# louislung/DAE_RNN_News_Recommendation

Measured on NVIDIA H100. Metric: articles/sec, higher is better.
Workload: dtype f32

## Files before the change

### dae_rnn_news_recommendation_b200/csrc/gemm_tc.cu

```cuda
#include <cuda.h>
#include <cuda_bf16.h>
#include <type_traits>
#include "common.cuh"

namespace dae {

constexpr int BLOCK_M = 128;
constexpr int BLOCK_K = 64;
constexpr int WGMMA_K = 16;
constexpr int kThreads = 384;
constexpr int kDecodeN = 128;

__device__ __forceinline__ uint32_t smem_u32(const void* p) { return (uint32_t)__cvta_generic_to_shared(p); }

__device__ __forceinline__ void mbar_init(uint64_t* bar, uint32_t count) {
  asm volatile("mbarrier.init.shared::cta.b64 [%0], %1;" ::"r"(smem_u32(bar)), "r"(count));
}
__device__ __forceinline__ void mbar_expect_tx(uint64_t* bar, uint32_t bytes) {
  asm volatile("mbarrier.arrive.expect_tx.shared::cta.b64 _, [%0], %1;" ::"r"(smem_u32(bar)), "r"(bytes) : "memory");
}
__device__ __forceinline__ void mbar_arrive(uint64_t* bar) {
  asm volatile("mbarrier.arrive.shared::cta.b64 _, [%0];" ::"r"(smem_u32(bar)) : "memory");
}
__device__ __forceinline__ bool mbar_try_wait(uint64_t* bar, uint32_t parity) {
  uint32_t ok;
  asm volatile(
      "{\n"
      ".reg .pred p;\n"
      "mbarrier.try_wait.parity.shared::cta.b64 p, [%1], %2;\n"
      "selp.u32 %0, 1, 0, p;\n"
      "}\n"
      : "=r"(ok)
      : "r"(smem_u32(bar)), "r"(parity)
      : "memory");
  return ok != 0;
}
__device__ __forceinline__ void mbar_wait(uint64_t* bar, uint32_t parity) {
  uint32_t spins = 0;
  while (!mbar_try_wait(bar, parity)) {
    if (++spins > 4096u) {
      __nanosleep(64);
      if (spins > (1u << 26)) __trap();
    }
  }
}
__device__ __forceinline__ void fence_barrier_init() { asm volatile("fence.mbarrier_init.release.cluster;" ::: "memory"); }

__device__ __forceinline__ void tma_load_2d(const CUtensorMap* map, uint64_t* bar, void* dst, int c0, int c1) {
  asm volatile(
      "cp.async.bulk.tensor.2d.shared::cluster.global.mbarrier::complete_tx::bytes [%0], [%1, {%3, %4}], [%2];" ::"r"(smem_u32(dst)),
      "l"(map), "r"(smem_u32(bar)), "r"(c0), "r"(c1)
      : "memory");
}
__device__ __forceinline__ uint32_t cluster_ctarank() { uint32_t r; asm volatile("mov.u32 %0, %%cluster_ctarank;" : "=r"(r)); return r; }
__device__ __forceinline__ void cluster_sync_all() {
  asm volatile("barrier.cluster.arrive.release.aligned;" ::: "memory");
  asm volatile("barrier.cluster.wait.acquire.aligned;" ::: "memory");
}
__device__ __forceinline__ void tma_load_2d_mc(const CUtensorMap* map, uint64_t* bar, void* dst, int c0, int c1, uint16_t cta_mask) {
  asm volatile(
      "cp.async.bulk.tensor.2d.shared::cluster.global.mbarrier::complete_tx::bytes.multicast::cluster [%0], [%1, {%3, %4}], [%2], %5;" ::"r"(
          smem_u32(dst)),
      "l"(map), "r"(smem_u32(bar)), "r"(c0), "r"(c1), "h"(cta_mask)
      : "memory");
}
__device__ __forceinline__ void mbar_arrive_cluster(uint64_t* bar, uint32_t rank) {
  uint32_t raddr;
  asm volatile("mapa.shared::cluster.u32 %0, %1, %2;" : "=r"(raddr) : "r"(smem_u32(bar)), "r"(rank));
  asm volatile("mbarrier.arrive.release.cluster.shared::cluster.b64 _, [%0];" ::"r"(raddr) : "memory");
}
__device__ __forceinline__ void mbar_wait_cluster(uint64_t* bar, uint32_t parity) {
  uint32_t spins = 0;
  for (;;) {
    uint32_t ok;
    asm volatile(
        "{\n"
        ".reg .pred p;\n"
        "mbarrier.try_wait.parity.acquire.cluster.shared::cta.b64 p, [%1], %2;\n"
        "selp.u32 %0, 1, 0, p;\n"
        "}\n"
        : "=r"(ok)
        : "r"(smem_u32(bar)), "r"(parity)
        : "memory");
    if (ok) return;
    if (++spins > 4096u) { __nanosleep(64); if (spins > (1u << 26)) __trap(); }
  }
}

__device__ __forceinline__ void prefetch_tmap(const CUtensorMap* map) {
  asm volatile("prefetch.tensormap [%0];" ::"l"(map) : "memory");
}
__device__ __forceinline__ void named_bar_sync(int id, int threads) { asm volatile("bar.sync %0, %1;" ::"r"(id), "r"(threads) : "memory"); }

__device__ __forceinline__ void wgmma_fence() { asm volatile("wgmma.fence.sync.aligned;" ::: "memory"); }
__device__ __forceinline__ void wgmma_commit() { asm volatile("wgmma.commit_group.sync.aligned;" ::: "memory"); }
template <int N>
__device__ __forceinline__ void wgmma_wait() { asm volatile("wgmma.wait_group.sync.aligned %0;" ::"n"(N) : "memory"); }

__device__ __forceinline__ uint64_t make_desc(uint32_t saddr, uint32_t lbo_bytes, uint32_t sbo_bytes) {
  uint64_t d = 0;
  d |= (uint64_t)((saddr >> 4) & 0x3FFF);
  d |= (uint64_t)((lbo_bytes >> 4) & 0x3FFF) << 16;
  d |= (uint64_t)((sbo_bytes >> 4) & 0x3FFF) << 32;
  d |= (uint64_t)1 << 62;
  return d;
}


template <int TA, int TB>
__device__ __forceinline__ void wgmma_n128(float (&d)[64], uint64_t da, uint64_t db, uint32_t scale_d) {
  asm volatile(
      "{\n"
      ".reg .pred p;\n"
      "setp.ne.b32 p, %66, 0;\n"
      "wgmma.mma_async.sync.aligned.m64n128k16.f32.bf16.bf16 "
      "{%0, %1, %2, %3, %4, %5, %6, %7, %8, %9, %10, %11, %12, %13, %14, %15, %16, %17, %18, %19, %20, %21, %22, %23, %24, %25, %26, %27, %28, %29, %30, %31, %32, %33, %34, %35, %36, %37, %38, %39, %40, %41, %42, %43, %44, %45, %46, %47, %48, %49, %50, %51, %52, %53, %54, %55, %56, %57, %58, %59, %60, %61, %62, %63}, %64, %65, p, 1, 1, %67, %68;\n"
      "}\n"
      : "+f"(d[0]), "+f"(d[1]), "+f"(d[2]), "+f"(d[3]), "+f"(d[4]), "+f"(d[5]), "+f"(d[6]), "+f"(d[7]), "+f"(d[8]), "+f"(d[9]), "+f"(d[10]), "+f"(d[11]), "+f"(d[12]), "+f"(d[13]), "+f"(d[14]), "+f"(d[15]), "+f"(d[16]), "+f"(d[17]), "+f"(d[18]), "+f"(d[19]), "+f"(d[20]), "+f"(d[21]), "+f"(d[22]), "+f"(d[23]), "+f"(d[24]), "+f"(d[25]), "+f"(d[26]), "+f"(d[27]), "+f"(d[28]), "+f"(d[29]), "+f"(d[30]), "+f"(d[31]), "+f"(d[32]), "+f"(d[33]), "+f"(d[34]), "+f"(d[35]), "+f"(d[36]), "+f"(d[37]), "+f"(d[38]), "+f"(d[39]), "+f"(d[40]), "+f"(d[41]), "+f"(d[42]), "+f"(d[43]), "+f"(d[44]), "+f"(d[45]), "+f"(d[46]), "+f"(d[47]), "+f"(d[48]), "+f"(d[49]), "+f"(d[50]), "+f"(d[51]), "+f"(d[52]), "+f"(d[53]), "+f"(d[54]), "+f"(d[55]), "+f"(d[56]), "+f"(d[57]), "+f"(d[58]), "+f"(d[59]), "+f"(d[60]), "+f"(d[61]), "+f"(d[62]), "+f"(d[63])
      : "l"(da), "l"(db), "r"(scale_d), "n"(TA), "n"(TB));
}

template <int TA, int TB>
__device__ __forceinline__ void wgmma_n64(float (&d)[32], uint64_t da, uint64_t db, uint32_t scale_d) {
  asm volatile(
      "{\n"
      ".reg .pred p;\n"
      "setp.ne.b32 p, %34, 0;\n"
      "wgmma.mma_async.sync.aligned.m64n64k16.f32.bf16.bf16 "
      "{%0, %1, %2, %3, %4, %5, %6, %7, %8, %9, %10, %11, %12, %13, %14, %15, %16, %17, %18, %19, %20, %21, %22, %23, %24, %25, %26, %27, %28, %29, %30, %31}, %32, %33, p, 1, 1, %35, %36;\n"
      "}\n"
      : "+f"(d[0]), "+f"(d[1]), "+f"(d[2]), "+f"(d[3]), "+f"(d[4]), "+f"(d[5]), "+f"(d[6]), "+f"(d[7]), "+f"(d[8]), "+f"(d[9]), "+f"(d[10]), "+f"(d[11]), "+f"(d[12]), "+f"(d[13]), "+f"(d[14]), "+f"(d[15]), "+f"(d[16]), "+f"(d[17]), "+f"(d[18]), "+f"(d[19]), "+f"(d[20]), "+f"(d[21]), "+f"(d[22]), "+f"(d[23]), "+f"(d[24]), "+f"(d[25]), "+f"(d[26]), "+f"(d[27]), "+f"(d[28]), "+f"(d[29]), "+f"(d[30]), "+f"(d[31])
      : "l"(da), "l"(db), "r"(scale_d), "n"(TA), "n"(TB));
}

struct GemmParams {
  int M, N, K;
  int k_splits;
  int stream_k;
  int atomic;
  int a_mn, b_mn;
  int a_sym_kb;
  float alpha;
  float* C;
  int64_t ldc;
  int n_store;
  int special_col;
  float* special_out;
  const int64_t* indptr; const int32_t* indices; const float* values; const int32_t* rows;
  const float* bv; const float* weight; const double* stats;
  __nv_bfloat16* dz_hi; __nv_bfloat16* dz_lo; int64_t ld_dz;
  float* row_loss_part;
  const int32_t* tile_ptr;
};

enum { EPI_STORE = 0, EPI_DECODE = 1 };

struct Sched {
  int tiles_m, tiles, kb_total, kb_per_split, n_work, stream, w, n_cta;
  long long u, u_end;
  __device__ __forceinline__ void init(const GemmParams& p, int block_n, int pair = 0) {
    const int cta = pair ? (int)(blockIdx.x >> 1) : (int)blockIdx.x;
    n_cta = pair ? (int)(gridDim.x >> 1) : (int)gridDim.x;
    tiles_m = (p.M + BLOCK_M - 1) / BLOCK_M;
    if (pair) tiles_m = (tiles_m + 1) / 2;
    tiles = tiles_m * ((p.N + block_n - 1) / block_n);
    kb_total = (p.K + BLOCK_K - 1) / BLOCK_K;
    stream = p.stream_k;
    kb_per_split = (kb_total + p.k_splits - 1) / p.k_splits;
    n_work = tiles * p.k_splits;
    w = cta;
    const long long U = (long long)tiles * kb_total;
    u = (long long)cta * U / n_cta;
    u_end = (long long)(cta + 1) * U / n_cta;
  }
  __device__ __forceinline__ bool next(int& mb, int& nb, int& kb0, int& kb1) {
    int tile;
    if (stream) {
      if (u >= u_end) return false;
      tile = (int)(u / kb_total);
      kb0 = (int)(u - (long long)tile * kb_total);
      const long long left = u_end - u;
      kb1 = (left < (long long)(kb_total - kb0)) ? kb0 + (int)left : kb_total;
      u += kb1 - kb0;
    } else {
      if (w >= n_work) return false;
      tile = w % tiles;
      kb0 = (w / tiles) * kb_per_split;
      kb1 = min(kb_total, kb0 + kb_per_split);
      w += n_cta;
    }
    mb = tile % tiles_m;
    nb = tile / tiles_m;
    return true;
  }
};

__device__ __forceinline__ uint32_t pack_bf16(float a, float b) {
  const __nv_bfloat162 v = __floats2bfloat162_rn(a, b);
  return *reinterpret_cast<const uint32_t*>(&v);
}
__device__ __forceinline__ float f_rcp(float x) { float r; asm("rcp.approx.ftz.f32 %0, %1;" : "=f"(r) : "f"(x)); return r; }
__device__ __forceinline__ float f_lg2(float x) { float r; asm("lg2.approx.ftz.f32 %0, %1;" : "=f"(r) : "f"(x)); return r; }
__device__ __forceinline__ float f_ex2(float x) { float r; asm("ex2.approx.ftz.f32 %0, %1;" : "=f"(r) : "f"(x)); return r; }
constexpr float kLog2e = 1.4426950408889634f;

template <int ACT>
__device__ __forceinline__ float act_fast(float z) {
  if (ACT == DAE_ACT_SIGMOID) return f_rcp(1.0f + f_ex2(-kLog2e * z));
  if (ACT == DAE_ACT_TANH) return 1.0f - 2.0f * f_rcp(1.0f + f_ex2(2.0f * kLog2e * z));
  return z;
}


__device__ __forceinline__ float select16(const uint32_t (&r)[16], int j) {
  uint32_t v = r[0];
#pragma unroll
  for (int k = 1; k < 16; ++k) v = (j == k) ? r[k] : v;
  return __uint_as_float(v);
}

template <int ACT, int LOSS>
__device__ __forceinline__ void decode_chunk_generic(const uint32_t (&r)[16], const float* __restrict__ bias, float sc, bool edge,
                                                     int n_lim, int nc, uint32_t (&hpk)[8], uint32_t (&lpk)[8], float& lsum) {
#pragma unroll
  for (int j2 = 0; j2 < 8; ++j2) {
    float dzp[2];
#pragma unroll
    for (int e = 0; e < 2; ++e) {
      const int j = 2 * j2 + e;
      const float z = __uint_as_float(r[j]) + bias[j];
      const float d = act_fast<ACT>(z);
      float dz, lt;
      if (LOSS == DAE_LOSS_CE) {
        const float omd = 1.0f - d;
        const float b = omd + kEps;
        lt = -f_lg2(b);
        dz = (ACT == DAE_ACT_SIGMOID) ? ((omd != 0.0f) ? sc * d : 0.0f) : sc * act_grad_from_y<ACT>(d) * f_rcp(b);
      } else {
        lt = d * d;
        dz = 2.0f * sc * d * act_grad_from_y<ACT>(d);
      }
      if (edge) { const bool in = (nc + j < n_lim); lt = in ? lt : 0.0f; dz = in ? dz : 0.0f; }
      lsum += lt;
      dzp[e] = dz;
    }
    const uint32_t hp = pack_bf16(dzp[0], dzp[1]);
    hpk[j2] = hp;
    lpk[j2] = pack_bf16(dzp[0] - __uint_as_float(hp << 16), dzp[1] - __uint_as_float(hp & 0xffff0000u));
  }
}

__device__ __forceinline__ bool decode_chunk_sigmoid_ce(const uint32_t (&r)[16], const float* __restrict__ biasc, float sc,
                                                        uint32_t (&hpk)[8], uint32_t (&lpk)[8], float& lsum) {
  bool ok = true;
#pragma unroll
  for (int g = 0; g < 4; ++g) {
    float t[4], a[4];
#pragma unroll
    for (int j = 0; j < 4; ++j) {
      t[j] = f_ex2(fmaf(__uint_as_float(r[4 * g + j]), kLog2e, biasc[4 * g + j]));
      a[j] = 1.0f + t[j];
    }
    const float p01 = a[0] * a[1], p23 = a[2] * a[3], P = p01 * p23;
    ok = ok && (P <= 22026.0f);
    const float Rs = f_rcp(P) * sc;
    lsum += f_lg2(P);
    const float r23 = Rs * p23, r01 = Rs * p01;
    const float dz0 = t[0] * (r23 * a[1]), dz1 = t[1] * (r23 * a[0]), dz2 = t[2] * (r01 * a[3]), dz3 = t[3] * (r01 * a[2]);
    const uint32_t h0 = pack_bf16(dz0, dz1), h1 = pack_bf16(dz2, dz3);
    hpk[2 * g] = h0; hpk[2 * g + 1] = h1;
    lpk[2 * g] = pack_bf16(dz0 - __uint_as_float(h0 << 16), dz1 - __uint_as_float(h0 & 0xffff0000u));
    lpk[2 * g + 1] = pack_bf16(dz2 - __uint_as_float(h1 << 16), dz3 - __uint_as_float(h1 & 0xffff0000u));
  }
  return ok;
}

template <int BLOCK_N, int TA, int TB>
__device__ __forceinline__ void mma_kblock(float (&acc)[BLOCK_N / 2], uint32_t sa_hi, uint32_t sa_lo, uint32_t sb_hi, uint32_t sb_lo,
                                           bool first) {
  constexpr uint32_t a_lbo = TA ? 8192u : 16u, b_lbo = TB ? 8192u : 16u;
  constexpr uint32_t a_step = TA ? 2048u : 32u, b_step = TB ? 2048u : 32u;
#pragma unroll
  for (int k = 0; k < BLOCK_K / WGMMA_K; ++k) {
    const uint64_t da_hi = make_desc(sa_hi + k * a_step, a_lbo, 1024), da_lo = make_desc(sa_lo + k * a_step, a_lbo, 1024);
    const uint64_t db_hi = make_desc(sb_hi + k * b_step, b_lbo, 1024), db_lo = make_desc(sb_lo + k * b_step, b_lbo, 1024);
    const uint32_t sc = (first && k == 0) ? 0u : 1u;
    if constexpr (BLOCK_N == 128) {
      wgmma_n128<TA, TB>(acc, da_lo, db_hi, sc);
      wgmma_n128<TA, TB>(acc, da_hi, db_lo, 1u);
      wgmma_n128<TA, TB>(acc, da_hi, db_hi, 1u);
    } else {
      wgmma_n64<TA, TB>(acc, da_lo, db_hi, sc);
      wgmma_n64<TA, TB>(acc, da_hi, db_lo, 1u);
      wgmma_n64<TA, TB>(acc, da_hi, db_hi, 1u);
    }
  }
}

__device__ __forceinline__ void stage_ld16(const float* src, uint32_t (&r)[16]) {
#pragma unroll
  for (int q = 0; q < 4; ++q) {
    const float4 v = reinterpret_cast<const float4*>(src)[q];
    r[4 * q] = __float_as_uint(v.x); r[4 * q + 1] = __float_as_uint(v.y); r[4 * q + 2] = __float_as_uint(v.z); r[4 * q + 3] = __float_as_uint(v.w);
  }
}

template <int BLOCK_N, int STAGES, int EPI, int ACT, int LOSS, int PAIR, int MAJ>
__global__ void __launch_bounds__(kThreads, 1) gemm_bf16x3_kernel(const __grid_constant__ CUtensorMap tm_a_hi,
                                                                   const __grid_constant__ CUtensorMap tm_a_lo,
                                                                   const __grid_constant__ CUtensorMap tm_b_hi,
                                                                   const __grid_constant__ CUtensorMap tm_b_lo,
                                                                   const __grid_constant__ CUtensorMap tm_at_hi,
                                                                   const __grid_constant__ CUtensorMap tm_at_lo,
                                                                   const GemmParams p) {
  static_assert(!PAIR || BLOCK_N == 128, "CTA pairs split the B tile into two 64-row halves");
  constexpr int A_TILE = BLOCK_M * BLOCK_K * 2;
  constexpr int B_TILE = BLOCK_N * BLOCK_K * 2;
  constexpr int STAGE_BYTES = 2 * A_TILE + 2 * B_TILE;
  constexpr int SROW = BLOCK_N + 4;
  constexpr int kParts = 2;
  constexpr int HALF_N = BLOCK_N / kParts;
  constexpr bool kFast = (EPI == EPI_DECODE) && (ACT == DAE_ACT_SIGMOID) && (LOSS == DAE_LOSS_CE);
  extern __shared__ __align__(1024) uint8_t smem_raw[];
  uint8_t* smem = reinterpret_cast<uint8_t*>((reinterpret_cast<uintptr_t>(smem_raw) + 1023) & ~(uintptr_t)1023);
  float* stg = reinterpret_cast<float*>(smem + STAGES * STAGE_BYTES);
  __shared__ __align__(8) uint64_t full_bar[STAGES], empty_bar[STAGES];
  __shared__ float s_bias[EPI == EPI_DECODE ? 2 : 1][EPI == EPI_DECODE ? BLOCK_N : 1];
  __shared__ float s_biasc[kFast ? 2 : 1][kFast ? BLOCK_N : 1];
  __shared__ __align__(16) uint8_t s_stage[EPI == EPI_DECODE ? 8 : 1][2][32][48];

  const int warp = threadIdx.x >> 5, lane = threadIdx.x & 31;
  Sched sched;
  sched.init(p, BLOCK_N, PAIR);
  const uint32_t crank = PAIR ? cluster_ctarank() : 0u;

  if (warp == 0 && lane == 0) {
    prefetch_tmap(&tm_a_hi); prefetch_tmap(&tm_a_lo); prefetch_tmap(&tm_b_hi); prefetch_tmap(&tm_b_lo);
    if (p.a_sym_kb > 0) { prefetch_tmap(&tm_at_hi); prefetch_tmap(&tm_at_lo); }
  }
  if (warp == 1 && lane == 0) {
    for (int s = 0; s < STAGES; ++s) { mbar_init(&full_bar[s], 1); mbar_init(&empty_bar[s], PAIR ? 16 : 8); }
    fence_barrier_init();
  }
  if (PAIR) cluster_sync_all(); else __syncthreads();

  if (warp == 0) {
    if (lane == 0) {
      int stage = 0; uint32_t phase = 0;
      int mb, nb, kb0, kb1;
      while (sched.next(mb, nb, kb0, kb1)) {
        for (int kb = kb0; kb < kb1; ++kb) {
          if (PAIR) mbar_wait_cluster(&empty_bar[stage], phase ^ 1); else mbar_wait(&empty_bar[stage], phase ^ 1);
          uint8_t* sa_hi = smem + stage * STAGE_BYTES;
          uint8_t* sa_lo = sa_hi + A_TILE;
          uint8_t* sb_hi = sa_lo + A_TILE;
          uint8_t* sb_lo = sb_hi + B_TILE;
          const int mt = PAIR ? mb * 2 + (int)crank : mb;
          mbar_expect_tx(&full_bar[stage], STAGE_BYTES);
          if (p.a_sym_kb > 0 && kb >= p.a_sym_kb) {
#pragma unroll
            for (int j = 0; j < BLOCK_M / 64; ++j) {
              tma_load_2d(&tm_at_hi, &full_bar[stage], sa_hi + j * 8192, mt * BLOCK_M + j * 64, (kb - p.a_sym_kb) * BLOCK_K);
              tma_load_2d(&tm_at_lo, &full_bar[stage], sa_lo + j * 8192, mt * BLOCK_M + j * 64, (kb - p.a_sym_kb) * BLOCK_K);
            }
          } else if (!p.a_mn) {
            tma_load_2d(&tm_a_hi, &full_bar[stage], sa_hi, kb * BLOCK_K, mt * BLOCK_M);
            tma_load_2d(&tm_a_lo, &full_bar[stage], sa_lo, kb * BLOCK_K, mt * BLOCK_M);
          } else {
#pragma unroll
            for (int j = 0; j < BLOCK_M / 64; ++j) {
              tma_load_2d(&tm_a_hi, &full_bar[stage], sa_hi + j * 8192, mt * BLOCK_M + j * 64, kb * BLOCK_K);
              tma_load_2d(&tm_a_lo, &full_bar[stage], sa_lo + j * 8192, mt * BLOCK_M + j * 64, kb * BLOCK_K);
            }
          }
          const int kbb = (p.a_sym_kb > 0 && kb >= p.a_sym_kb) ? kb - p.a_sym_kb : kb;
          if (PAIR) {
            const int off = (int)crank * 8192, n_half = nb * BLOCK_N + (int)crank * 64;
            if (!p.b_mn) {
              tma_load_2d_mc(&tm_b_hi, &full_bar[stage], sb_hi + off, kbb * BLOCK_K, n_half, 0x3);
              tma_load_2d_mc(&tm_b_lo, &full_bar[stage], sb_lo + off, kbb * BLOCK_K, n_half, 0x3);
            } else {
              tma_load_2d_mc(&tm_b_hi, &full_bar[stage], sb_hi + off, n_half, kbb * BLOCK_K, 0x3);
              tma_load_2d_mc(&tm_b_lo, &full_bar[stage], sb_lo + off, n_half, kbb * BLOCK_K, 0x3);
            }
          } else if (!p.b_mn) {
            tma_load_2d(&tm_b_hi, &full_bar[stage], sb_hi, kbb * BLOCK_K, nb * BLOCK_N);
            tma_load_2d(&tm_b_lo, &full_bar[stage], sb_lo, kbb * BLOCK_K, nb * BLOCK_N);
          } else {
#pragma unroll
            for (int j = 0; j < BLOCK_N / 64; ++j) {
              tma_load_2d(&tm_b_hi, &full_bar[stage], sb_hi + j * 8192, nb * BLOCK_N + j * 64, kbb * BLOCK_K);
              tma_load_2d(&tm_b_lo, &full_bar[stage], sb_lo + j * 8192, nb * BLOCK_N + j * 64, kbb * BLOCK_K);
            }
          }
          if (++stage == STAGES) { stage = 0; phase ^= 1; }
        }
      }
    }
  } else if (warp >= 4) {
    const int wg = (warp >> 2) - 1;
    const int wi = warp & 3;
    const int quarter = wg * 2 + (wi & 1);
    const int half = wi >> 1;
    const int row_in_tile = quarter * 32 + lane;
    const int tiles_n = (p.N + BLOCK_N - 1) / BLOCK_N;
    float acc[BLOCK_N / 2];
#pragma unroll
    for (int i = 0; i < BLOCK_N / 2; ++i) acc[i] = 0.0f;
    int stage = 0; uint32_t phase = 0;
    auto release = [&](int s) {
      __syncwarp();
      if (lane == 0) { mbar_arrive(&empty_bar[s]); if (PAIR) mbar_arrive_cluster(&empty_bar[s], crank ^ 1u); }
    };
    int mb, nb, kb0, kb1;
    while (sched.next(mb, nb, kb0, kb1)) {
      if (PAIR) mb = mb * 2 + (int)crank;
      int prev = -1;
      auto run_k = [&](auto ta, auto tb, int kb_begin, int kb_end) {
        for (int kb = kb_begin; kb < kb_end; ++kb) {
          mbar_wait(&full_bar[stage], phase);
          const uint32_t sa_hi = smem_u32(smem + stage * STAGE_BYTES) + wg * 8192;
          const uint32_t sa_lo = sa_hi + A_TILE;
          const uint32_t sb_hi = smem_u32(smem + stage * STAGE_BYTES) + 2 * A_TILE, sb_lo = sb_hi + B_TILE;
          wgmma_fence();
          mma_kblock<BLOCK_N, decltype(ta)::value, decltype(tb)::value>(acc, sa_hi, sa_lo, sb_hi, sb_lo, kb == kb0);
          wgmma_commit();
          wgmma_wait<1>();
          if (prev >= 0) release(prev);
          prev = stage;
          if (++stage == STAGES) { stage = 0; phase ^= 1; }
        }
      };
      using K0 = std::integral_constant<int, 0>;
      using K1 = std::integral_constant<int, 1>;
      if (MAJ & 4) {
        run_k(K0{}, K1{}, kb0, min(kb1, p.a_sym_kb));
        run_k(K1{}, K1{}, max(kb0, p.a_sym_kb), kb1);
      } else {
        run_k(std::integral_constant<int, MAJ & 1>{}, std::integral_constant<int, (MAJ >> 1) & 1>{}, kb0, kb1);
      }
      wgmma_wait<0>();
      if (prev >= 0) release(prev);

      named_bar_sync(1 + wg, 128);
      {
        const int r0 = wg * 64 + wi * 16 + (lane >> 2), c0 = 2 * (lane & 3);
#pragma unroll
        for (int j = 0; j < BLOCK_N / 8; ++j) {
          *reinterpret_cast<float2*>(&stg[r0 * SROW + 8 * j + c0]) = make_float2(acc[4 * j], acc[4 * j + 1]);
          *reinterpret_cast<float2*>(&stg[(r0 + 8) * SROW + 8 * j + c0]) = make_float2(acc[4 * j + 2], acc[4 * j + 3]);
        }
      }
      if (EPI == EPI_DECODE) {
        for (int j = threadIdx.x - 128 * (wg + 1); j < BLOCK_N; j += 128) {
          const float b = (nb * BLOCK_N + j < p.N) ? p.bv[nb * BLOCK_N + j] : 0.0f;
          s_bias[wg][j] = b;
          if (kFast) s_biasc[wg][j] = b * kLog2e;
        }
      }
      named_bar_sync(1 + wg, 128);
      const float* srow = stg + row_in_tile * SROW + half * HALF_N;
      const int m = mb * BLOCK_M + row_in_tile;
      const int n0 = nb * BLOCK_N + half * HALF_N;

      if (EPI == EPI_STORE) {
        const float* tr = stg + (quarter * 32) * SROW + half * HALF_N;
        const int m_base = mb * BLOCK_M + quarter * 32;
        const bool vec_ok = ((p.ldc & 3) == 0) && ((reinterpret_cast<uintptr_t>(p.C) & 15) == 0);
#pragma unroll 1
        for (int c = 0; c < HALF_N / 16; ++c) {
          const int nc = n0 + c * 16;
          const bool interior = vec_ok && (m_base + 32 <= p.M) && (nc + 16 <= p.n_store) && (p.special_col < nc || p.special_col >= nc + 16);
          if (interior) {
            const int rsub = lane >> 2, c4 = (lane & 3) * 4;
            float* dst = p.C + (int64_t)(m_base + rsub) * p.ldc + nc + c4;
            const int64_t step = 8 * p.ldc;
#pragma unroll
            for (int i = 0; i < 4; ++i) {
              float4 v = *reinterpret_cast<const float4*>(&tr[(rsub + 8 * i) * SROW + c * 16 + c4]);
              v.x *= p.alpha; v.y *= p.alpha; v.z *= p.alpha; v.w *= p.alpha;
              if (p.atomic) atomicAdd(reinterpret_cast<float4*>(dst), v); else *reinterpret_cast<float4*>(dst) = v;
              dst += step;
            }
          } else {
            const int rsub = lane >> 4, csub = lane & 15;
            const int n = nc + csub;
            for (int i = 0; i < 16; ++i) {
              const int rr = 2 * i + rsub;
              const int mm = m_base + rr;
              const float v = p.alpha * tr[rr * SROW + c * 16 + csub];
              if (mm < p.M) {
                if (n == p.special_col) {
                  if (p.atomic) atomicAdd(p.special_out + mm, v); else p.special_out[mm] = v;
                } else if (n < p.n_store) {
                  float* dst = p.C + (int64_t)mm * p.ldc + n;
                  if (p.atomic) atomicAdd(dst, v); else *dst = v;
                }
              }
            }
          }
        }
      } else {
        int64_t pc = 0, pe = 0;
        int c0 = 0x7fffffff, c1 = 0x7fffffff, c2 = 0x7fffffff;
        float v0 = 0.0f, v1 = 0.0f, v2 = 0.0f;
        float sc = 0.0f;
        if (m < p.M) {
          const int64_t row = p.rows ? (int64_t)p.rows[m] : (int64_t)m;
          const int64_t rbeg = p.indptr[row];
          const int32_t* tp = p.tile_ptr + (int64_t)m * (kParts * tiles_n + 1) + nb * kParts + half;
          pc = rbeg + tp[0]; pe = rbeg + tp[1];
          if (pc < pe) { c0 = p.indices[pc]; v0 = p.values[pc]; }
          if (pc + 1 < pe) { c1 = p.indices[pc + 1]; v1 = p.values[pc + 1]; }
          if (pc + 2 < pe) { c2 = p.indices[pc + 2]; v2 = p.values[pc + 2]; }
          sc = (p.weight ? p.weight[m] : 1.0f) / ((float)p.stats[DAE_STAT_SUM_W] + kEps);
        }
        const float inv_sc = (sc != 0.0f) ? 1.0f / sc : 0.0f;
        const bool edge = (n0 + HALF_N > p.N);
        float lsum = 0.0f;
        const int ew = warp - 4;
        uint8_t* stg_hi = reinterpret_cast<uint8_t*>(&s_stage[ew][0][0][0]);
        uint8_t* stg_lo = reinterpret_cast<uint8_t*>(&s_stage[ew][1][0][0]);
        const int rsub = lane >> 1, csub = lane & 1;
        const int m_base = mb * BLOCK_M + quarter * 32;
        const int n_lim = edge ? p.N : 0x7fffffff;
#pragma unroll 1
        for (int c = 0; c < HALF_N / 16; ++c) {
          uint32_t r[16];
          stage_ld16(srow + c * 16, r);
          const int nc = n0 + c * 16;
          if (m < p.M) {
            const float* bias = &s_bias[wg][half * HALF_N + c * 16];
            uint32_t hpk[8], lpk[8];
            bool fast_ok = false;
            if (kFast && !edge) {
              const float l0 = lsum;
              fast_ok = decode_chunk_sigmoid_ce(r, &s_biasc[wg][half * HALF_N + c * 16], sc, hpk, lpk, lsum);
              if (!fast_ok) { lsum = l0; decode_chunk_generic<ACT, LOSS>(r, bias, sc, edge, n_lim, nc, hpk, lpk, lsum); }
            } else {
              decode_chunk_generic<ACT, LOSS>(r, bias, sc, edge, n_lim, nc, hpk, lpk, lsum);
            }
            uint4* sh = reinterpret_cast<uint4*>(stg_hi + lane * 48);
            uint4* sl = reinterpret_cast<uint4*>(stg_lo + lane * 48);
            sh[0] = make_uint4(hpk[0], hpk[1], hpk[2], hpk[3]); sh[1] = make_uint4(hpk[4], hpk[5], hpk[6], hpk[7]);
            sl[0] = make_uint4(lpk[0], lpk[1], lpk[2], lpk[3]); sl[1] = make_uint4(lpk[4], lpk[5], lpk[6], lpk[7]);
            while (c0 < nc + 16) {
              const float x = v0;
              const int j = c0 - nc;
              __nv_bfloat16* ph = reinterpret_cast<__nv_bfloat16*>(stg_hi + lane * 48) + j;
              __nv_bfloat16* pl = reinterpret_cast<__nv_bfloat16*>(stg_lo + lane * 48) + j;
              float d;
              if (kFast && fast_ok && sc != 0.0f) d = (__bfloat162float(*ph) + __bfloat162float(*pl)) * inv_sc;
              else d = act_fast<ACT>(select16(r, j) + bias[j]);
              const float gp = act_grad_from_y<ACT>(d);
              float dz;
              if (LOSS == DAE_LOSS_CE) {
                const float a = d + kEps, b = (1.0f - d) + kEps;
                const float la = f_lg2(a), lb = f_lg2(b);
                lsum += lb - (x * la + (1.0f - x) * lb);
                dz = sc * gp * ((1.0f - x) * f_rcp(b) - x * f_rcp(a));
              } else {
                const float e2 = x - d;
                lsum += e2 * e2 - d * d;
                dz = -2.0f * sc * e2 * gp;
              }
              const __nv_bfloat16 hb = __float2bfloat16_rn(dz);
              *ph = hb;
              *pl = __float2bfloat16_rn(dz - __bfloat162float(hb));
              ++pc;
              c0 = c1; v0 = v1; c1 = c2; v1 = v2;
              c2 = 0x7fffffff;
              if (pc + 2 < pe) { c2 = p.indices[pc + 2]; v2 = p.values[pc + 2]; }
            }
          }
          __syncwarp();
          if (nc < p.ld_dz) {
#pragma unroll
            for (int i = 0; i < 2; ++i) {
              const int rr = rsub + 16 * i;
              if (m_base + rr < p.M) {
                const int64_t off = (int64_t)(m_base + rr) * p.ld_dz + nc + csub * 8;
                *reinterpret_cast<uint4*>(p.dz_hi + off) = *reinterpret_cast<const uint4*>(stg_hi + rr * 48 + csub * 16);
                *reinterpret_cast<uint4*>(p.dz_lo + off) = *reinterpret_cast<const uint4*>(stg_lo + rr * 48 + csub * 16);
              }
            }
          }
          __syncwarp();
        }
        if (m < p.M) atomicAdd(p.row_loss_part + m, (LOSS == DAE_LOSS_CE) ? lsum * 0.6931471805599453f : lsum);
      }
    }
  }

  if (PAIR) cluster_sync_all();
}

__global__ void decode_tile_ptr_kernel(const int64_t* __restrict__ indptr, const int32_t* __restrict__ indices,
                                       const int32_t* __restrict__ rows, int M, int n_half_tiles, int half_n,
                                       int32_t* __restrict__ tile_ptr) {
  const int t = blockIdx.x * blockDim.x + threadIdx.x;
  const int m = blockIdx.y;
  if (t > n_half_tiles || m >= M) return;
  const int64_t row = rows ? (int64_t)rows[m] : (int64_t)m;
  const int64_t b = indptr[row], e = indptr[row + 1];
  const int target = t * half_n;
  int64_t lo = b, hi = e;
  while (lo < hi) { const int64_t mid = (lo + hi) >> 1; if (indices[mid] < target) lo = mid + 1; else hi = mid; }
  tile_ptr[(int64_t)m * (n_half_tiles + 1) + t] = (int32_t)(lo - b);
}

__global__ void split_bf16_kernel(const float* __restrict__ src, int rows, int cols, int64_t ld_src, __nv_bfloat16* __restrict__ hi,
                                  __nv_bfloat16* __restrict__ lo, int64_t ld_dst, int ones_col, float scale) {
  const int64_t total = (int64_t)rows * ld_dst;
  for (int64_t i = (int64_t)blockIdx.x * blockDim.x + threadIdx.x; i < total; i += (int64_t)gridDim.x * blockDim.x) {
    const int64_t r = i / ld_dst;
    const int c = (int)(i - r * ld_dst);
    float v = (c < cols) ? src[r * ld_src + c] * scale : 0.0f;
    if (c == ones_col) v = 1.0f;
    const __nv_bfloat16 h = __float2bfloat16_rn(v);
    hi[i] = h;
    lo[i] = __float2bfloat16_rn(v - __bfloat162float(h));
  }
}

__global__ void sym_split_kernel(const float* __restrict__ G, int B, int64_t ldg, float alpha, __nv_bfloat16* __restrict__ hi,
                                 __nv_bfloat16* __restrict__ lo, int64_t ld) {
  __shared__ float t[32][33];
  const int bx = blockIdx.x * 32, by = blockIdx.y * 32;
  const int tx = threadIdx.x, ty = threadIdx.y;
  for (int j = ty; j < 32; j += 8) {
    const int r = bx + j, c = by + tx;
    t[j][tx] = (r < B && c < B) ? G[(int64_t)r * ldg + c] : 0.0f;
  }
  __syncthreads();
  for (int j = ty; j < 32; j += 8) {
    const int r = by + j, c = bx + tx;
    if (r < B && c < ld) {
      float v = 0.0f;
      if (c < B) v = alpha * (G[(int64_t)r * ldg + c] + t[tx][j]);
      const __nv_bfloat16 h = __float2bfloat16_rn(v);
      hi[(int64_t)r * ld + c] = h;
      lo[(int64_t)r * ld + c] = __float2bfloat16_rn(v - __bfloat162float(h));
    }
  }
}

typedef CUresult (*PFN_encodeTiled)(CUtensorMap*, CUtensorMapDataType, cuuint32_t, void*, const cuuint64_t*, const cuuint64_t*,
                                    const cuuint32_t*, const cuuint32_t*, CUtensorMapInterleave, CUtensorMapSwizzle,
                                    CUtensorMapL2promotion, CUtensorMapFloatOOBfill);

static PFN_encodeTiled get_encode() {
  static PFN_encodeTiled fn = nullptr;
  if (!fn) {
    void* sym = nullptr;
    cudaDriverEntryPointQueryResult q;
    if (cudaGetDriverEntryPoint("cuTensorMapEncodeTiled", &sym, cudaEnableDefault, &q) == cudaSuccess && q == cudaDriverEntryPointSuccess)
      fn = reinterpret_cast<PFN_encodeTiled>(sym);
  }
  return fn;
}

static int make_map(CUtensorMap* m, const void* base, uint64_t inner, uint64_t outer, uint64_t ld, uint32_t box_outer) {
  PFN_encodeTiled enc = get_encode();
  if (!enc) { set_error("cuTensorMapEncodeTiled entry point not found"); return DAE_ERR_CUDA; }
  cuuint64_t dims[2] = {inner, outer};
  cuuint64_t strides[1] = {ld * 2};
  cuuint32_t box[2] = {64, box_outer};
  cuuint32_t estr[2] = {1, 1};
  CUresult r = enc(m, CU_TENSOR_MAP_DATA_TYPE_BFLOAT16, 2, const_cast<void*>(base), dims, strides, box, estr,
                   CU_TENSOR_MAP_INTERLEAVE_NONE, CU_TENSOR_MAP_SWIZZLE_128B, CU_TENSOR_MAP_L2_PROMOTION_L2_256B,
                   CU_TENSOR_MAP_FLOAT_OOB_FILL_NONE);
  if (r != CUDA_SUCCESS) { set_error("cuTensorMapEncodeTiled failed (%d): inner=%llu outer=%llu ld=%llu", (int)r,
                                     (unsigned long long)inner, (unsigned long long)outer, (unsigned long long)ld); return DAE_ERR_CUDA; }
  return DAE_OK;
}

struct Operand { const void* hi; const void* lo; int64_t ld; int mn_major; };

template <typename Kern>
static int ensure_smem_attr(Kern kern, int smem, bool (&done)[64]) {
  int dev = 0;
  DAE_CUDA(cudaGetDevice(&dev));
  if (dev < 0 || dev >= 64 || !done[dev]) {
    DAE_CUDA(cudaFuncSetAttribute(kern, cudaFuncAttributeMaxDynamicSharedMemorySize, smem));
    if (dev >= 0 && dev < 64) done[dev] = true;
  }
  return DAE_OK;
}


static int g_pair_mode = -1;
static int g_lean = 0;

template <int BLOCK_N, int STAGES, int EPI, int ACT, int LOSS, int PAIR, int MAJ>
static int launch_gemm_maj(const Operand& A, const Operand& B, GemmParams p, cudaStream_t st) {
  CUtensorMap ta_hi, ta_lo, tb_hi, tb_lo;
  int rc;
  constexpr int B_ROWS = PAIR ? BLOCK_N / 2 : BLOCK_N;
  if (!A.mn_major) {
    const uint64_t a_cols = p.a_sym_kb > 0 ? (uint64_t)p.M : (uint64_t)p.K;
    if ((rc = make_map(&ta_hi, A.hi, a_cols, p.M, A.ld, BLOCK_M))) return rc;
    if ((rc = make_map(&ta_lo, A.lo, a_cols, p.M, A.ld, BLOCK_M))) return rc;
  } else {
    if ((rc = make_map(&ta_hi, A.hi, p.M, p.K, A.ld, 64))) return rc;
    if ((rc = make_map(&ta_lo, A.lo, p.M, p.K, A.ld, 64))) return rc;
  }
  if (!B.mn_major) {
    if ((rc = make_map(&tb_hi, B.hi, p.K, p.N, B.ld, B_ROWS))) return rc;
    if ((rc = make_map(&tb_lo, B.lo, p.K, p.N, B.ld, B_ROWS))) return rc;
  } else {
    const uint64_t b_rows = p.a_sym_kb > 0 ? (uint64_t)p.M : (uint64_t)p.K;
    if ((rc = make_map(&tb_hi, B.hi, p.N, b_rows, B.ld, 64))) return rc;
    if ((rc = make_map(&tb_lo, B.lo, p.N, b_rows, B.ld, 64))) return rc;
  }
  p.a_mn = A.mn_major; p.b_mn = B.mn_major;
  CUtensorMap tat_hi = ta_hi, tat_lo = ta_lo;
  if (p.a_sym_kb > 0) {
    if (PAIR || A.mn_major) { set_error("dae_gemm_sym_bf16x3: unsupported configuration"); return DAE_ERR_UNSUPPORTED; }
    if ((rc = make_map(&tat_hi, A.hi, p.M, p.M, A.ld, 64))) return rc;
    if ((rc = make_map(&tat_lo, A.lo, p.M, p.M, A.ld, 64))) return rc;
  }
  constexpr int smem = STAGES * (2 * BLOCK_M * BLOCK_K * 2 + 2 * BLOCK_N * BLOCK_K * 2) + BLOCK_M * (BLOCK_N + 4) * 4 + 1024;
  int tiles_m = (p.M + BLOCK_M - 1) / BLOCK_M;
  if (PAIR) tiles_m = (tiles_m + 1) / 2;
  const int tiles_n = (p.N + BLOCK_N - 1) / BLOCK_N;
  const int kblocks = (p.K + BLOCK_K - 1) / BLOCK_K;
  auto kern = gemm_bf16x3_kernel<BLOCK_N, STAGES, EPI, ACT, LOSS, PAIR, MAJ>;
  static bool attr_done[64] = {false};
  if ((rc = ensure_smem_attr(kern, smem, attr_done))) return rc;
  const int slots = PAIR ? sm_count() / 2 : sm_count();
  int n;
  if (p.stream_k) {
    const long long units = (long long)tiles_m * tiles_n * kblocks;
    long long g = units / 6;
    if (g < 1) g = 1;
    n = (int)(g < slots ? g : slots);
  } else {
    const int items = tiles_m * tiles_n * p.k_splits;
    n = items < slots ? items : slots;
  }
  if (!PAIR) {
    kern<<<n, kThreads, smem, st>>>(ta_hi, ta_lo, tb_hi, tb_lo, tat_hi, tat_lo, p);
  } else {
    cudaLaunchConfig_t cfg{};
    cfg.gridDim = dim3(2 * n); cfg.blockDim = dim3(kThreads); cfg.dynamicSmemBytes = smem; cfg.stream = st;
    cudaLaunchAttribute at[1];
    at[0].id = cudaLaunchAttributeClusterDimension;
    at[0].val.clusterDim.x = 2; at[0].val.clusterDim.y = 1; at[0].val.clusterDim.z = 1;
    cfg.attrs = at; cfg.numAttrs = 1;
    DAE_CUDA(cudaLaunchKernelEx(&cfg, kern, ta_hi, ta_lo, tb_hi, tb_lo, tat_hi, tat_lo, p));
  }
  return DAE_OK;
}

template <int BLOCK_N, int STAGES, int EPI, int ACT, int LOSS, int PAIR>
static int launch_gemm(const Operand& A, const Operand& B, GemmParams p, cudaStream_t st) {
  if (EPI == EPI_DECODE || (!A.mn_major && !B.mn_major)) return launch_gemm_maj<BLOCK_N, STAGES, EPI, ACT, LOSS, PAIR, 0>(A, B, p, st);
  if constexpr (EPI == EPI_STORE) {
    if (A.mn_major && !B.mn_major) return launch_gemm_maj<BLOCK_N, STAGES, EPI, ACT, LOSS, PAIR, 1>(A, B, p, st);
    if (!A.mn_major) return launch_gemm_maj<BLOCK_N, STAGES, EPI, ACT, LOSS, PAIR, 2>(A, B, p, st);
    return launch_gemm_maj<BLOCK_N, STAGES, EPI, ACT, LOSS, PAIR, 3>(A, B, p, st);
  }
  return DAE_ERR_UNSUPPORTED;
}

static bool use_pair() { return g_pair_mode == 1 && !g_lean; }

}

using namespace dae;

extern "C" int dae_split_bf16(const float* src, int32_t rows, int32_t cols, int64_t ld_src, void* hi, void* lo, int64_t ld_dst,
                              int32_t ones_col, float scale, void* stream) {
  DAE_REQUIRE(src && hi && lo && rows > 0 && cols > 0 && ld_src >= cols && ld_dst >= cols, "dae_split_bf16: bad arguments");
  const int64_t total = (int64_t)rows * ld_dst;
  const int cap = sm_count() * 16;
  const int blocks = (int)((total + 255) / 256 < cap ? (total + 255) / 256 : cap);
  split_bf16_kernel<<<blocks, 256, 0, (cudaStream_t)stream>>>(src, rows, cols, ld_src, (__nv_bfloat16*)hi, (__nv_bfloat16*)lo, ld_dst,
                                                              ones_col, scale);
  DAE_CHECK_LAUNCH("dae_split_bf16");
  return DAE_OK;
}

extern "C" int dae_sym_split_bf16(const float* G, int32_t B, int64_t ldg, float alpha, void* hi, void* lo, int64_t ld, void* stream) {
  DAE_REQUIRE(G && hi && lo && B > 0 && ldg >= B && ld >= B, "dae_sym_split_bf16: bad arguments");
  dim3 grid((unsigned)((ld + 31) / 32), (B + 31) / 32), block(32, 8);
  sym_split_kernel<<<grid, block, 0, (cudaStream_t)stream>>>(G, B, ldg, alpha, (__nv_bfloat16*)hi, (__nv_bfloat16*)lo, ld);
  DAE_CHECK_LAUNCH("dae_sym_split_bf16");
  return DAE_OK;
}

extern "C" int dae_gemm_config(int32_t pair_mode, int32_t lean) {
  dae::g_pair_mode = pair_mode < 0 ? -1 : (pair_mode ? 1 : 0);
  dae::g_lean = lean ? 1 : 0;
  return DAE_OK;
}

extern "C" int dae_gemm_bf16x3(int32_t M, int32_t N, int32_t K, float alpha, const void* a_hi, const void* a_lo, int64_t lda,
                               int32_t a_mn_major, const void* b_hi, const void* b_lo, int64_t ldb, int32_t b_mn_major, float* C,
                               int64_t ldc, int32_t n_store, int32_t special_col, float* special_out, int32_t k_splits,
                               int32_t accumulate, void* stream) {
  DAE_REQUIRE(a_hi && a_lo && b_hi && b_lo && C && M > 0 && N > 0 && K > 0, "dae_gemm_bf16x3: bad arguments");
  DAE_REQUIRE(lda % 8 == 0 && ldb % 8 == 0, "dae_gemm_bf16x3: operand leading dimensions must be multiples of 8 (TMA 16-byte strides)");
  DAE_REQUIRE(((uintptr_t)a_hi | (uintptr_t)a_lo | (uintptr_t)b_hi | (uintptr_t)b_lo) % 16 == 0, "dae_gemm_bf16x3: operands must be 16-byte aligned");
  cudaStream_t st = (cudaStream_t)stream;
  if (n_store <= 0 || n_store > N) n_store = N;
  const int kblocks = (K + BLOCK_K - 1) / BLOCK_K;
  const int tm = (M + 127) / 128, tn128 = (N + 127) / 128, tn64 = (N + 63) / 64;
  const int sms = sm_count();
  int stream_k = 0;
  if (k_splits < 0) {
    const int t = tm * tn128;
    stream_k = (t % sms == 0) ? 0 : 1;
    k_splits = 1;
  }
  if (k_splits < 1) k_splits = 1;
  if (k_splits > kblocks) k_splits = kblocks;
  {
    const int per = (kblocks + k_splits - 1) / k_splits;
    k_splits = (kblocks + per - 1) / per;
  }
  const bool partial = (k_splits > 1) || stream_k;
  if (partial && !accumulate) {
    DAE_CUDA(cudaMemset2DAsync(C, ldc * sizeof(float), 0, (size_t)n_store * sizeof(float), M, st));
    if (special_col >= 0 && special_out) DAE_CUDA(cudaMemsetAsync(special_out, 0, sizeof(float) * M, st));
  }
  GemmParams p{};
  p.M = M; p.N = N; p.K = K; p.k_splits = k_splits; p.stream_k = stream_k; p.atomic = (partial || accumulate) ? 1 : 0; p.alpha = alpha;
  p.C = C; p.ldc = ldc; p.n_store = n_store;
  p.special_col = (special_out ? special_col : -1); p.special_out = special_out;
  Operand A{a_hi, a_lo, lda, a_mn_major}, B{b_hi, b_lo, ldb, b_mn_major};
  int rc;
  const int tiles128 = tm * tn128 * k_splits, tiles64 = tm * tn64 * k_splits;
  const float cost128 = 2.0f * (float)((tiles128 + sms - 1) / sms), cost64 = 1.1f * (float)((tiles64 + sms - 1) / sms);
  if (g_lean) rc = launch_gemm<64, 2, EPI_STORE, 0, 0, 0>(A, B, p, st);
  else if (use_pair()) rc = launch_gemm<128, 2, EPI_STORE, 0, 0, 1>(A, B, p, st);
  else if (!stream_k && cost64 < cost128) rc = launch_gemm<64, 3, EPI_STORE, 0, 0, 0>(A, B, p, st);
  else rc = launch_gemm<128, 2, EPI_STORE, 0, 0, 0>(A, B, p, st);
  if (rc) return rc;
  DAE_CHECK_LAUNCH("dae_gemm_bf16x3");
  return DAE_OK;
}

extern "C" int dae_gemm_sym_bf16x3(int32_t M, int32_t N, float alpha, const void* g_hi, const void* g_lo, int64_t ldg, const void* b_hi,
                                   const void* b_lo, int64_t ldb, float* C, int64_t ldc, int32_t accumulate, void* stream) {
  DAE_REQUIRE(g_hi && g_lo && b_hi && b_lo && C && M > 0 && N > 0, "dae_gemm_sym_bf16x3: bad arguments");
  DAE_REQUIRE(ldg % 8 == 0 && ldb % 8 == 0 && ldg >= M && ldb >= N, "dae_gemm_sym_bf16x3: leading dimensions must be multiples of 8 and cover the matrices");
  DAE_REQUIRE(((uintptr_t)g_hi | (uintptr_t)g_lo | (uintptr_t)b_hi | (uintptr_t)b_lo) % 16 == 0, "dae_gemm_sym_bf16x3: operands must be 16-byte aligned");
  GemmParams p{};
  const int kb_half = (M + BLOCK_K - 1) / BLOCK_K;
  p.M = M; p.N = N; p.K = 2 * kb_half * BLOCK_K; p.k_splits = 1; p.stream_k = 1; p.atomic = 1; p.alpha = alpha;
  p.C = C; p.ldc = ldc; p.n_store = N; p.special_col = -1; p.special_out = nullptr; p.a_sym_kb = kb_half;
  if (!accumulate) DAE_CUDA(cudaMemset2DAsync(C, ldc * sizeof(float), 0, (size_t)N * sizeof(float), M, (cudaStream_t)stream));
  Operand A{g_hi, g_lo, ldg, 0}, B{b_hi, b_lo, ldb, 1};
  int rc = launch_gemm_maj<128, 2, EPI_STORE, 0, 0, 0, 6>(A, B, p, (cudaStream_t)stream);
  if (rc) return rc;
  DAE_CHECK_LAUNCH("dae_gemm_sym_bf16x3");
  return DAE_OK;
}

extern "C" int dae_decode_prepare(int32_t Brows, int32_t F, const int64_t* indptr, const int32_t* indices, const int32_t* rows,
                                  float* row_loss_part, int32_t* tile_ptr, void* stream) {
  DAE_REQUIRE(Brows > 0 && F > 0 && indptr && indices && row_loss_part && tile_ptr, "dae_decode_prepare: bad arguments");
  cudaStream_t st = (cudaStream_t)stream;
  DAE_CUDA(cudaMemsetAsync(row_loss_part, 0, sizeof(float) * Brows, st));
  const int n_half = 2 * ((F + kDecodeN - 1) / kDecodeN);
  dim3 grid((n_half + 1 + 127) / 128, Brows);
  decode_tile_ptr_kernel<<<grid, 128, 0, st>>>(indptr, indices, rows, Brows, n_half, kDecodeN / 2, tile_ptr);
  DAE_CHECK_LAUNCH("dae_decode_prepare");
  return DAE_OK;
}

extern "C" int dae_decode_fused_bf16x3(int32_t Brows, int32_t F, int32_t K, const void* e_hi, const void* e_lo, int64_t lde,
                                       const void* w_hi, const void* w_lo, int64_t ldw, const int64_t* indptr, const int32_t* indices,
                                       const float* values, const int32_t* rows, const float* bv, int32_t dec_act, int32_t loss_func,
                                       const float* weight, const double* stats, void* dz_hi, void* dz_lo, int64_t ld_dz,
                                       float* row_loss_part, int32_t* tile_ptr, int32_t prepared, void* stream) {
  DAE_REQUIRE(e_hi && e_lo && w_hi && w_lo && indptr && indices && values && bv && stats && dz_hi && dz_lo && row_loss_part && tile_ptr,
              "dae_decode_fused_bf16x3: null pointer");
  DAE_REQUIRE(loss_func == DAE_LOSS_CE || loss_func == DAE_LOSS_MSE, "dae_decode_fused_bf16x3: cosine loss uses the unfused path");
  DAE_REQUIRE(lde % 8 == 0 && ldw % 8 == 0 && ld_dz % 32 == 0 && ld_dz >= F, "dae_decode_fused_bf16x3: bad leading dimensions");
  cudaStream_t st = (cudaStream_t)stream;
  GemmParams p{};
  p.M = Brows; p.N = F; p.K = K; p.k_splits = 1; p.alpha = 1.0f; p.special_col = -1;
  p.indptr = indptr; p.indices = indices; p.values = values; p.rows = rows; p.bv = bv; p.weight = weight; p.stats = stats;
  p.dz_hi = (__nv_bfloat16*)dz_hi; p.dz_lo = (__nv_bfloat16*)dz_lo; p.ld_dz = ld_dz; p.row_loss_part = row_loss_part;
  p.tile_ptr = tile_ptr;
  if (!prepared) {
    int rc0 = dae_decode_prepare(Brows, F, indptr, indices, rows, row_loss_part, tile_ptr, stream);
    if (rc0) return rc0;
  }
  Operand A{e_hi, e_lo, lde, 0}, B{w_hi, w_lo, ldw, 0};
  int rc = 0;
  const bool pair = (g_pair_mode == 1);
#define DAE_DEC(ACT, LOSS) rc = pair ? launch_gemm<kDecodeN, 2, EPI_DECODE, ACT, LOSS, 1>(A, B, p, st) \
                              : launch_gemm<kDecodeN, 2, EPI_DECODE, ACT, LOSS, 0>(A, B, p, st)
  if (loss_func == DAE_LOSS_CE) {
    if (dec_act == DAE_ACT_SIGMOID) DAE_DEC(DAE_ACT_SIGMOID, DAE_LOSS_CE);
    else if (dec_act == DAE_ACT_TANH) DAE_DEC(DAE_ACT_TANH, DAE_LOSS_CE);
    else DAE_DEC(DAE_ACT_NONE, DAE_LOSS_CE);
  } else {
    if (dec_act == DAE_ACT_SIGMOID) DAE_DEC(DAE_ACT_SIGMOID, DAE_LOSS_MSE);
    else if (dec_act == DAE_ACT_TANH) DAE_DEC(DAE_ACT_TANH, DAE_LOSS_MSE);
    else DAE_DEC(DAE_ACT_NONE, DAE_LOSS_MSE);
  }
#undef DAE_DEC
  if (rc) return rc;
  DAE_CHECK_LAUNCH("dae_decode_fused_bf16x3");
  return DAE_OK;
}
```

Before: 2.060 million.

## Split fused decode into dedicated kernel with 32-wide k-blocks and overlapped epilogue

Moves the decode epilogue out of the generic GEMM kernel into a dedicated decode_fused_kernel. The new kernel uses 32-wide k-blocks with 64B-swizzled TMA maps and more stages, and appears to double-buffer accumulators with a drained barrier so the epilogue of one tile can overlap the MMA of the next. The producer and MMA loops are factored into shared helpers parameterised by k-block width. The aim is to hide the heavy sparse-loss epilogue behind tensor-core work, at the cost of extra shared memory, dropping the CTA-pair path for decode, and more barrier complexity.

```diff
diff --git a/dae_rnn_news_recommendation_b200/csrc/gemm_tc.cu b/dae_rnn_news_recommendation_b200/csrc/gemm_tc.cu
--- a/dae_rnn_news_recommendation_b200/csrc/gemm_tc.cu
+++ b/dae_rnn_news_recommendation_b200/csrc/gemm_tc.cu
@@ -97,12 +97,12 @@
 template <int N>
 __device__ __forceinline__ void wgmma_wait() { asm volatile("wgmma.wait_group.sync.aligned %0;" ::"n"(N) : "memory"); }
 
-__device__ __forceinline__ uint64_t make_desc(uint32_t saddr, uint32_t lbo_bytes, uint32_t sbo_bytes) {
+__device__ __forceinline__ uint64_t make_desc(uint32_t saddr, uint32_t lbo_bytes, uint32_t sbo_bytes, uint32_t layout = 1) {
   uint64_t d = 0;
   d |= (uint64_t)((saddr >> 4) & 0x3FFF);
   d |= (uint64_t)((lbo_bytes >> 4) & 0x3FFF) << 16;
   d |= (uint64_t)((sbo_bytes >> 4) & 0x3FFF) << 32;
-  d |= (uint64_t)1 << 62;
+  d |= (uint64_t)layout << 62;
   return d;
 }
 
@@ -153,18 +153,16 @@
   const int32_t* tile_ptr;
 };
 
-enum { EPI_STORE = 0, EPI_DECODE = 1 };
-
 struct Sched {
   int tiles_m, tiles, kb_total, kb_per_split, n_work, stream, w, n_cta;
   long long u, u_end;
-  __device__ __forceinline__ void init(const GemmParams& p, int block_n, int pair = 0) {
+  __device__ __forceinline__ void init(const GemmParams& p, int block_n, int pair = 0, int block_k = BLOCK_K) {
     const int cta = pair ? (int)(blockIdx.x >> 1) : (int)blockIdx.x;
     n_cta = pair ? (int)(gridDim.x >> 1) : (int)gridDim.x;
     tiles_m = (p.M + BLOCK_M - 1) / BLOCK_M;
     if (pair) tiles_m = (tiles_m + 1) / 2;
     tiles = tiles_m * ((p.N + block_n - 1) / block_n);
-    kb_total = (p.K + BLOCK_K - 1) / BLOCK_K;
+    kb_total = (p.K + block_k - 1) / block_k;
     stream = p.stream_k;
     kb_per_split = (kb_total + p.k_splits - 1) / p.k_splits;
     n_work = tiles * p.k_splits;
@@ -275,15 +273,17 @@
   return ok;
 }
 
-template <int BLOCK_N, int TA, int TB>
+template <int BLOCK_N, int TA, int TB, int BK = BLOCK_K>
 __device__ __forceinline__ void mma_kblock(float (&acc)[BLOCK_N / 2], uint32_t sa_hi, uint32_t sa_lo, uint32_t sb_hi, uint32_t sb_lo,
                                            bool first) {
+  static_assert(BK == 64 || (BK == 32 && !TA && !TB), "32-wide k-blocks are K-major only");
+  constexpr uint32_t layout = BK == 64 ? 1u : 2u, sbo = BK == 64 ? 1024u : 512u;
   constexpr uint32_t a_lbo = TA ? 8192u : 16u, b_lbo = TB ? 8192u : 16u;
   constexpr uint32_t a_step = TA ? 2048u : 32u, b_step = TB ? 2048u : 32u;
 #pragma unroll
-  for (int k = 0; k < BLOCK_K / WGMMA_K; ++k) {
-    const uint64_t da_hi = make_desc(sa_hi + k * a_step, a_lbo, 1024), da_lo = make_desc(sa_lo + k * a_step, a_lbo, 1024);
-    const uint64_t db_hi = make_desc(sb_hi + k * b_step, b_lbo, 1024), db_lo = make_desc(sb_lo + k * b_step, b_lbo, 1024);
+  for (int k = 0; k < BK / WGMMA_K; ++k) {
+    const uint64_t da_hi = make_desc(sa_hi + k * a_step, a_lbo, sbo, layout), da_lo = make_desc(sa_lo + k * a_step, a_lbo, sbo, layout);
+    const uint64_t db_hi = make_desc(sb_hi + k * b_step, b_lbo, sbo, layout), db_lo = make_desc(sb_lo + k * b_step, b_lbo, sbo, layout);
     const uint32_t sc = (first && k == 0) ? 0u : 1u;
     if constexpr (BLOCK_N == 128) {
       wgmma_n128<TA, TB>(acc, da_lo, db_hi, sc);
@@ -305,7 +305,107 @@
   }
 }
 
-template <int BLOCK_N, int STAGES, int EPI, int ACT, int LOSS, int PAIR, int MAJ>
+
+template <int BLOCK_N, int STAGES, int PAIR, int BK = BLOCK_K>
+__device__ __forceinline__ void tma_produce(const GemmParams& p, Sched& sched, uint8_t* smem, uint64_t* full_bar, uint64_t* empty_bar,
+                                            uint32_t crank, const CUtensorMap* tm_a_hi, const CUtensorMap* tm_a_lo,
+                                            const CUtensorMap* tm_b_hi, const CUtensorMap* tm_b_lo, const CUtensorMap* tm_at_hi,
+                                            const CUtensorMap* tm_at_lo) {
+  constexpr int A_TILE = BLOCK_M * BK * 2;
+  constexpr int B_TILE = BLOCK_N * BK * 2;
+  constexpr int STAGE_BYTES = 2 * A_TILE + 2 * B_TILE;
+  int stage = 0; uint32_t phase = 0;
+  int mb, nb, kb0, kb1;
+  while (sched.next(mb, nb, kb0, kb1)) {
+    for (int kb = kb0; kb < kb1; ++kb) {
+      if (PAIR) mbar_wait_cluster(&empty_bar[stage], phase ^ 1); else mbar_wait(&empty_bar[stage], phase ^ 1);
+      uint8_t* sa_hi = smem + stage * STAGE_BYTES;
+      uint8_t* sa_lo = sa_hi + A_TILE;
+      uint8_t* sb_hi = sa_lo + A_TILE;
+      uint8_t* sb_lo = sb_hi + B_TILE;
+      const int mt = PAIR ? mb * 2 + (int)crank : mb;
+      mbar_expect_tx(&full_bar[stage], STAGE_BYTES);
+      if (p.a_sym_kb > 0 && kb >= p.a_sym_kb) {
+#pragma unroll
+        for (int j = 0; j < BLOCK_M / 64; ++j) {
+          tma_load_2d(tm_at_hi, &full_bar[stage], sa_hi + j * (64 * BK * 2), mt * BLOCK_M + j * 64, (kb - p.a_sym_kb) * BK);
+          tma_load_2d(tm_at_lo, &full_bar[stage], sa_lo + j * (64 * BK * 2), mt * BLOCK_M + j * 64, (kb - p.a_sym_kb) * BK);
+        }
+      } else if (!p.a_mn) {
+        tma_load_2d(tm_a_hi, &full_bar[stage], sa_hi, kb * BK, mt * BLOCK_M);
+        tma_load_2d(tm_a_lo, &full_bar[stage], sa_lo, kb * BK, mt * BLOCK_M);
+      } else {
+#pragma unroll
+        for (int j = 0; j < BLOCK_M / 64; ++j) {
+          tma_load_2d(tm_a_hi, &full_bar[stage], sa_hi + j * (64 * BK * 2), mt * BLOCK_M + j * 64, kb * BK);
+          tma_load_2d(tm_a_lo, &full_bar[stage], sa_lo + j * (64 * BK * 2), mt * BLOCK_M + j * 64, kb * BK);
+        }
+      }
+      const int kbb = (p.a_sym_kb > 0 && kb >= p.a_sym_kb) ? kb - p.a_sym_kb : kb;
+      if (PAIR) {
+        const int off = (int)crank * 8192, n_half = nb * BLOCK_N + (int)crank * 64;
+        if (!p.b_mn) {
+          tma_load_2d_mc(tm_b_hi, &full_bar[stage], sb_hi + off, kbb * BK, n_half, 0x3);
+          tma_load_2d_mc(tm_b_lo, &full_bar[stage], sb_lo + off, kbb * BK, n_half, 0x3);
+        } else {
+          tma_load_2d_mc(tm_b_hi, &full_bar[stage], sb_hi + off, n_half, kbb * BK, 0x3);
+          tma_load_2d_mc(tm_b_lo, &full_bar[stage], sb_lo + off, n_half, kbb * BK, 0x3);
+        }
+      } else if (!p.b_mn) {
+        tma_load_2d(tm_b_hi, &full_bar[stage], sb_hi, kbb * BK, nb * BLOCK_N);
+        tma_load_2d(tm_b_lo, &full_bar[stage], sb_lo, kbb * BK, nb * BLOCK_N);
+      } else {
+#pragma unroll
+        for (int j = 0; j < BLOCK_N / 64; ++j) {
+          tma_load_2d(tm_b_hi, &full_bar[stage], sb_hi + j * (64 * BK * 2), nb * BLOCK_N + j * 64, kbb * BK);
+          tma_load_2d(tm_b_lo, &full_bar[stage], sb_lo + j * (64 * BK * 2), nb * BLOCK_N + j * 64, kbb * BK);
+        }
+      }
+      if (++stage == STAGES) { stage = 0; phase ^= 1; }
+    }
+  }
+}
+
+template <int BLOCK_N, int STAGES, int PAIR, int MAJ, int BK = BLOCK_K>
+__device__ __forceinline__ void mma_work_item(float (&acc)[BLOCK_N / 2], const GemmParams& p, uint8_t* smem, uint64_t* full_bar,
+                                              uint64_t* empty_bar, int wg, int lane, uint32_t crank, int& stage, uint32_t& phase,
+                                              int kb0, int kb1) {
+  constexpr int A_TILE = BLOCK_M * BK * 2;
+  constexpr int B_TILE = BLOCK_N * BK * 2;
+  constexpr int STAGE_BYTES = 2 * A_TILE + 2 * B_TILE;
+  auto release = [&](int s) {
+    __syncwarp();
+    if (lane == 0) { mbar_arrive(&empty_bar[s]); if (PAIR) mbar_arrive_cluster(&empty_bar[s], crank ^ 1u); }
+  };
+  int prev = -1;
+  auto run_k = [&](auto ta, auto tb, int kb_begin, int kb_end) {
+    for (int kb = kb_begin; kb < kb_end; ++kb) {
+      mbar_wait(&full_bar[stage], phase);
+      const uint32_t sa_hi = smem_u32(smem + stage * STAGE_BYTES) + wg * (64 * BK * 2);
+      const uint32_t sa_lo = sa_hi + A_TILE;
+      const uint32_t sb_hi = smem_u32(smem + stage * STAGE_BYTES) + 2 * A_TILE, sb_lo = sb_hi + B_TILE;
+      wgmma_fence();
+      mma_kblock<BLOCK_N, decltype(ta)::value, decltype(tb)::value, BK>(acc, sa_hi, sa_lo, sb_hi, sb_lo, kb == kb0);
+      wgmma_commit();
+      wgmma_wait<1>();
+      if (prev >= 0) release(prev);
+      prev = stage;
+      if (++stage == STAGES) { stage = 0; phase ^= 1; }
+    }
+  };
+  using K0 = std::integral_constant<int, 0>;
+  using K1 = std::integral_constant<int, 1>;
+  if constexpr ((MAJ & 4) != 0) {
+    run_k(K0{}, K1{}, kb0, min(kb1, p.a_sym_kb));
+    run_k(K1{}, K1{}, max(kb0, p.a_sym_kb), kb1);
+  } else {
+    run_k(std::integral_constant<int, MAJ & 1>{}, std::integral_constant<int, (MAJ >> 1) & 1>{}, kb0, kb1);
+  }
+  wgmma_wait<0>();
+  if (prev >= 0) release(prev);
+}
+
+template <int BLOCK_N, int STAGES, int PAIR, int MAJ>
 __global__ void __launch_bounds__(kThreads, 1) gemm_bf16x3_kernel(const __grid_constant__ CUtensorMap tm_a_hi,
                                                                    const __grid_constant__ CUtensorMap tm_a_lo,
                                                                    const __grid_constant__ CUtensorMap tm_b_hi,
@@ -314,20 +414,14 @@
                                                                    const __grid_constant__ CUtensorMap tm_at_lo,
                                                                    const GemmParams p) {
   static_assert(!PAIR || BLOCK_N == 128, "CTA pairs split the B tile into two 64-row halves");
-  constexpr int A_TILE = BLOCK_M * BLOCK_K * 2;
-  constexpr int B_TILE = BLOCK_N * BLOCK_K * 2;
-  constexpr int STAGE_BYTES = 2 * A_TILE + 2 * B_TILE;
+  constexpr int STAGE_BYTES = 2 * BLOCK_M * BLOCK_K * 2 + 2 * BLOCK_N * BLOCK_K * 2;
   constexpr int SROW = BLOCK_N + 4;
   constexpr int kParts = 2;
   constexpr int HALF_N = BLOCK_N / kParts;
-  constexpr bool kFast = (EPI == EPI_DECODE) && (ACT == DAE_ACT_SIGMOID) && (LOSS == DAE_LOSS_CE);
   extern __shared__ __align__(1024) uint8_t smem_raw[];
   uint8_t* smem = reinterpret_cast<uint8_t*>((reinterpret_cast<uintptr_t>(smem_raw) + 1023) & ~(uintptr_t)1023);
   float* stg = reinterpret_cast<float*>(smem + STAGES * STAGE_BYTES);
   __shared__ __align__(8) uint64_t full_bar[STAGES], empty_bar[STAGES];
-  __shared__ float s_bias[EPI == EPI_DECODE ? 2 : 1][EPI == EPI_DECODE ? BLOCK_N : 1];
-  __shared__ float s_biasc[kFast ? 2 : 1][kFast ? BLOCK_N : 1];
-  __shared__ __align__(16) uint8_t s_stage[EPI == EPI_DECODE ? 8 : 1][2][32][48];
 
   const int warp = threadIdx.x >> 5, lane = threadIdx.x & 31;
   Sched sched;
@@ -345,102 +439,22 @@
   if (PAIR) cluster_sync_all(); else __syncthreads();
 
   if (warp == 0) {
-    if (lane == 0) {
-      int stage = 0; uint32_t phase = 0;
-      int mb, nb, kb0, kb1;
-      while (sched.next(mb, nb, kb0, kb1)) {
-        for (int kb = kb0; kb < kb1; ++kb) {
-          if (PAIR) mbar_wait_cluster(&empty_bar[stage], phase ^ 1); else mbar_wait(&empty_bar[stage], phase ^ 1);
-          uint8_t* sa_hi = smem + stage * STAGE_BYTES;
-          uint8_t* sa_lo = sa_hi + A_TILE;
-          uint8_t* sb_hi = sa_lo + A_TILE;
-          uint8_t* sb_lo = sb_hi + B_TILE;
-          const int mt = PAIR ? mb * 2 + (int)crank : mb;
-          mbar_expect_tx(&full_bar[stage], STAGE_BYTES);
-          if (p.a_sym_kb > 0 && kb >= p.a_sym_kb) {
-#pragma unroll
-            for (int j = 0; j < BLOCK_M / 64; ++j) {
-              tma_load_2d(&tm_at_hi, &full_bar[stage], sa_hi + j * 8192, mt * BLOCK_M + j * 64, (kb - p.a_sym_kb) * BLOCK_K);
-              tma_load_2d(&tm_at_lo, &full_bar[stage], sa_lo + j * 8192, mt * BLOCK_M + j * 64, (kb - p.a_sym_kb) * BLOCK_K);
-            }
-          } else if (!p.a_mn) {
-            tma_load_2d(&tm_a_hi, &full_bar[stage], sa_hi, kb * BLOCK_K, mt * BLOCK_M);
-            tma_load_2d(&tm_a_lo, &full_bar[stage], sa_lo, kb * BLOCK_K, mt * BLOCK_M);
-          } else {
-#pragma unroll
-            for (int j = 0; j < BLOCK_M / 64; ++j) {
-              tma_load_2d(&tm_a_hi, &full_bar[stage], sa_hi + j * 8192, mt * BLOCK_M + j * 64, kb * BLOCK_K);
-              tma_load_2d(&tm_a_lo, &full_bar[stage], sa_lo + j * 8192, mt * BLOCK_M + j * 64, kb * BLOCK_K);
-            }
-          }
-          const int kbb = (p.a_sym_kb > 0 && kb >= p.a_sym_kb) ? kb - p.a_sym_kb : kb;
-          if (PAIR) {
-            const int off = (int)crank * 8192, n_half = nb * BLOCK_N + (int)crank * 64;
-            if (!p.b_mn) {
-              tma_load_2d_mc(&tm_b_hi, &full_bar[stage], sb_hi + off, kbb * BLOCK_K, n_half, 0x3);
-              tma_load_2d_mc(&tm_b_lo, &full_bar[stage], sb_lo + off, kbb * BLOCK_K, n_half, 0x3);
-            } else {
-              tma_load_2d_mc(&tm_b_hi, &full_bar[stage], sb_hi + off, n_half, kbb * BLOCK_K, 0x3);
-              tma_load_2d_mc(&tm_b_lo, &full_bar[stage], sb_lo + off, n_half, kbb * BLOCK_K, 0x3);
-            }
-          } else if (!p.b_mn) {
-            tma_load_2d(&tm_b_hi, &full_bar[stage], sb_hi, kbb * BLOCK_K, nb * BLOCK_N);
-            tma_load_2d(&tm_b_lo, &full_bar[stage], sb_lo, kbb * BLOCK_K, nb * BLOCK_N);
-          } else {
-#pragma unroll
-            for (int j = 0; j < BLOCK_N / 64; ++j) {
-              tma_load_2d(&tm_b_hi, &full_bar[stage], sb_hi + j * 8192, nb * BLOCK_N + j * 64, kbb * BLOCK_K);
-              tma_load_2d(&tm_b_lo, &full_bar[stage], sb_lo + j * 8192, nb * BLOCK_N + j * 64, kbb * BLOCK_K);
-            }
-          }
-          if (++stage == STAGES) { stage = 0; phase ^= 1; }
-        }
-      }
-    }
+    if (lane == 0)
+      tma_produce<BLOCK_N, STAGES, PAIR>(p, sched, smem, full_bar, empty_bar, crank, &tm_a_hi, &tm_a_lo, &tm_b_hi, &tm_b_lo, &tm_at_hi,
+                                         &tm_at_lo);
   } else if (warp >= 4) {
     const int wg = (warp >> 2) - 1;
     const int wi = warp & 3;
     const int quarter = wg * 2 + (wi & 1);
     const int half = wi >> 1;
-    const int row_in_tile = quarter * 32 + lane;
-    const int tiles_n = (p.N + BLOCK_N - 1) / BLOCK_N;
     float acc[BLOCK_N / 2];
 #pragma unroll
     for (int i = 0; i < BLOCK_N / 2; ++i) acc[i] = 0.0f;
     int stage = 0; uint32_t phase = 0;
-    auto release = [&](int s) {
-      __syncwarp();
-      if (lane == 0) { mbar_arrive(&empty_bar[s]); if (PAIR) mbar_arrive_cluster(&empty_bar[s], crank ^ 1u); }
-    };
     int mb, nb, kb0, kb1;
     while (sched.next(mb, nb, kb0, kb1)) {
       if (PAIR) mb = mb * 2 + (int)crank;
-      int prev = -1;
-      auto run_k = [&](auto ta, auto tb, int kb_begin, int kb_end) {
-        for (int kb = kb_begin; kb < kb_end; ++kb) {
-          mbar_wait(&full_bar[stage], phase);
-          const uint32_t sa_hi = smem_u32(smem + stage * STAGE_BYTES) + wg * 8192;
-          const uint32_t sa_lo = sa_hi + A_TILE;
-          const uint32_t sb_hi = smem_u32(smem + stage * STAGE_BYTES) + 2 * A_TILE, sb_lo = sb_hi + B_TILE;
-          wgmma_fence();
-          mma_kblock<BLOCK_N, decltype(ta)::value, decltype(tb)::value>(acc, sa_hi, sa_lo, sb_hi, sb_lo, kb == kb0);
-          wgmma_commit();
-          wgmma_wait<1>();
-          if (prev >= 0) release(prev);
-          prev = stage;
-          if (++stage == STAGES) { stage = 0; phase ^= 1; }
-        }
-      };
-      using K0 = std::integral_constant<int, 0>;
-      using K1 = std::integral_constant<int, 1>;
-      if (MAJ & 4) {
-        run_k(K0{}, K1{}, kb0, min(kb1, p.a_sym_kb));
-        run_k(K1{}, K1{}, max(kb0, p.a_sym_kb), kb1);
-      } else {
-        run_k(std::integral_constant<int, MAJ & 1>{}, std::integral_constant<int, (MAJ >> 1) & 1>{}, kb0, kb1);
-      }
-      wgmma_wait<0>();
-      if (prev >= 0) release(prev);
+      mma_work_item<BLOCK_N, STAGES, PAIR, MAJ>(acc, p, smem, full_bar, empty_bar, wg, lane, crank, stage, phase, kb0, kb1);
 
       named_bar_sync(1 + wg, 128);
       {
@@ -451,148 +465,234 @@
           *reinterpret_cast<float2*>(&stg[(r0 + 8) * SROW + 8 * j + c0]) = make_float2(acc[4 * j + 2], acc[4 * j + 3]);
         }
       }
-      if (EPI == EPI_DECODE) {
-        for (int j = threadIdx.x - 128 * (wg + 1); j < BLOCK_N; j += 128) {
-          const float b = (nb * BLOCK_N + j < p.N) ? p.bv[nb * BLOCK_N + j] : 0.0f;
-          s_bias[wg][j] = b;
-          if (kFast) s_biasc[wg][j] = b * kLog2e;
-        }
-      }
       named_bar_sync(1 + wg, 128);
-      const float* srow = stg + row_in_tile * SROW + half * HALF_N;
-      const int m = mb * BLOCK_M + row_in_tile;
       const int n0 = nb * BLOCK_N + half * HALF_N;
-
-      if (EPI == EPI_STORE) {
-        const float* tr = stg + (quarter * 32) * SROW + half * HALF_N;
-        const int m_base = mb * BLOCK_M + quarter * 32;
-        const bool vec_ok = ((p.ldc & 3) == 0) && ((reinterpret_cast<uintptr_t>(p.C) & 15) == 0);
+      const float* tr = stg + (quarter * 32) * SROW + half * HALF_N;
+      const int m_base = mb * BLOCK_M + quarter * 32;
+      const bool vec_ok = ((p.ldc & 3) == 0) && ((reinterpret_cast<uintptr_t>(p.C) & 15) == 0);
 #pragma unroll 1
-        for (int c = 0; c < HALF_N / 16; ++c) {
-          const int nc = n0 + c * 16;
-          const bool interior = vec_ok && (m_base + 32 <= p.M) && (nc + 16 <= p.n_store) && (p.special_col < nc || p.special_col >= nc + 16);
-          if (interior) {
-            const int rsub = lane >> 2, c4 = (lane & 3) * 4;
-            float* dst = p.C + (int64_t)(m_base + rsub) * p.ldc + nc + c4;
-            const int64_t step = 8 * p.ldc;
-#pragma unroll
-            for (int i = 0; i < 4; ++i) {
-              float4 v = *reinterpret_cast<const float4*>(&tr[(rsub + 8 * i) * SROW + c * 16 + c4]);
-              v.x *= p.alpha; v.y *= p.alpha; v.z *= p.alpha; v.w *= p.alpha;
-              if (p.atomic) atomicAdd(reinterpret_cast<float4*>(dst), v); else *reinterpret_cast<float4*>(dst) = v;
-              dst += step;
-            }
-          } else {
-            const int rsub = lane >> 4, csub = lane & 15;
-            const int n = nc + csub;
-            for (int i = 0; i < 16; ++i) {
-              const int rr = 2 * i + rsub;
-              const int mm = m_base + rr;
-              const float v = p.alpha * tr[rr * SROW + c * 16 + csub];
-              if (mm < p.M) {
-                if (n == p.special_col) {
-                  if (p.atomic) atomicAdd(p.special_out + mm, v); else p.special_out[mm] = v;
-                } else if (n < p.n_store) {
-                  float* dst = p.C + (int64_t)mm * p.ldc + n;
-                  if (p.atomic) atomicAdd(dst, v); else *dst = v;
-                }
+      for (int c = 0; c < HALF_N / 16; ++c) {
+        const int nc = n0 + c * 16;
+        const bool interior = vec_ok && (m_base + 32 <= p.M) && (nc + 16 <= p.n_store) && (p.special_col < nc || p.special_col >= nc + 16);
+        if (interior) {
+          const int rsub = lane >> 2, c4 = (lane & 3) * 4;
+          float* dst = p.C + (int64_t)(m_base + rsub) * p.ldc + nc + c4;
+          const int64_t step = 8 * p.ldc;
+#pragma unroll
+          for (int i = 0; i < 4; ++i) {
+            float4 v = *reinterpret_cast<const float4*>(&tr[(rsub + 8 * i) * SROW + c * 16 + c4]);
+            v.x *= p.alpha; v.y *= p.alpha; v.z *= p.alpha; v.w *= p.alpha;
+            if (p.atomic) atomicAdd(reinterpret_cast<float4*>(dst), v); else *reinterpret_cast<float4*>(dst) = v;
+            dst += step;
+          }
+        } else {
+          const int rsub = lane >> 4, csub = lane & 15;
+          const int n = nc + csub;
+          for (int i = 0; i < 16; ++i) {
+            const int rr = 2 * i + rsub;
+            const int mm = m_base + rr;
+            const float v = p.alpha * tr[rr * SROW + c * 16 + csub];
+            if (mm < p.M) {
+              if (n == p.special_col) {
+                if (p.atomic) atomicAdd(p.special_out + mm, v); else p.special_out[mm] = v;
+              } else if (n < p.n_store) {
+                float* dst = p.C + (int64_t)mm * p.ldc + n;
+                if (p.atomic) atomicAdd(dst, v); else *dst = v;
               }
             }
           }
         }
-      } else {
-        int64_t pc = 0, pe = 0;
-        int c0 = 0x7fffffff, c1 = 0x7fffffff, c2 = 0x7fffffff;
-        float v0 = 0.0f, v1 = 0.0f, v2 = 0.0f;
-        float sc = 0.0f;
+      }
+    }
+  }
+
+  if (PAIR) cluster_sync_all();
+}
+
+constexpr int kDecodeThreads = 640;
+constexpr int kDecodeBK = 32;
+constexpr int kDecodeStages = 4;
+constexpr int kRegsProducer = 32, kRegsMma = 104, kRegsEpilogue = 120;
+static_assert(128 * kRegsProducer + 256 * kRegsMma + 256 * kRegsEpilogue <= kDecodeThreads * 96, "register budget");
+
+template <int R> __device__ __forceinline__ void regs_dec() { asm volatile("setmaxnreg.dec.sync.aligned.u32 %0;" ::"n"(R)); }
+template <int R> __device__ __forceinline__ void regs_inc() { asm volatile("setmaxnreg.inc.sync.aligned.u32 %0;" ::"n"(R)); }
+
+template <int ACT, int LOSS>
+__global__ void __launch_bounds__(kDecodeThreads, 1) decode_fused_kernel(const __grid_constant__ CUtensorMap tm_a_hi,
+                                                                         const __grid_constant__ CUtensorMap tm_a_lo,
+                                                                         const __grid_constant__ CUtensorMap tm_b_hi,
+                                                                         const __grid_constant__ CUtensorMap tm_b_lo,
+                                                                         const GemmParams p) {
+  constexpr int BLOCK_N = kDecodeN, STAGES = kDecodeStages, BK = kDecodeBK;
+  constexpr int STAGE_BYTES = 2 * BLOCK_M * BK * 2 + 2 * BLOCK_N * BK * 2;
+  constexpr int SROW = BLOCK_N + 4;
+  constexpr int kParts = 2;
+  constexpr int HALF_N = BLOCK_N / kParts;
+  constexpr bool kFast = (ACT == DAE_ACT_SIGMOID) && (LOSS == DAE_LOSS_CE);
+  extern __shared__ __align__(1024) uint8_t smem_raw[];
+  uint8_t* smem = reinterpret_cast<uint8_t*>((reinterpret_cast<uintptr_t>(smem_raw) + 1023) & ~(uintptr_t)1023);
+  float* stg = reinterpret_cast<float*>(smem + STAGES * STAGE_BYTES);
+  __shared__ __align__(8) uint64_t full_bar[STAGES], empty_bar[STAGES], staged_bar[2], drained_bar[2];
+  __shared__ float s_bias[2][BLOCK_N];
+  __shared__ float s_biasc[kFast ? 2 : 1][kFast ? BLOCK_N : 1];
+  __shared__ __align__(16) uint8_t s_stage[8][2][32][48];
+
+  const int warp = threadIdx.x >> 5, lane = threadIdx.x & 31;
+  const int role = warp >> 2;
+  Sched sched;
+
+  if (warp == 0 && lane == 0) { prefetch_tmap(&tm_a_hi); prefetch_tmap(&tm_a_lo); prefetch_tmap(&tm_b_hi); prefetch_tmap(&tm_b_lo); }
+  if (warp == 1 && lane == 0) {
+    for (int s = 0; s < STAGES; ++s) { mbar_init(&full_bar[s], 1); mbar_init(&empty_bar[s], 8); }
+    for (int h = 0; h < 2; ++h) { mbar_init(&staged_bar[h], 4); mbar_init(&drained_bar[h], 4); }
+    fence_barrier_init();
+  }
+  __syncthreads();
+
+  if (role == 0) {
+    regs_dec<kRegsProducer>();
+    sched.init(p, BLOCK_N, 0, BK);
+    if (warp == 0 && lane == 0)
+      tma_produce<BLOCK_N, STAGES, 0, BK>(p, sched, smem, full_bar, empty_bar, 0u, &tm_a_hi, &tm_a_lo, &tm_b_hi, &tm_b_lo, &tm_a_hi, &tm_a_lo);
+  } else if (role <= 2) {
+    regs_inc<kRegsMma>();
+    sched.init(p, BLOCK_N, 0, BK);
+    const int h = role - 1;
+    const int wi = warp & 3;
+    float acc[BLOCK_N / 2];
+#pragma unroll
+    for (int i = 0; i < BLOCK_N / 2; ++i) acc[i] = 0.0f;
+    int stage = 0; uint32_t phase = 0, tphase = 0;
+    int mb, nb, kb0, kb1;
+    while (sched.next(mb, nb, kb0, kb1)) {
+      mma_work_item<BLOCK_N, STAGES, 0, 0, BK>(acc, p, smem, full_bar, empty_bar, h, lane, 0u, stage, phase, kb0, kb1);
+      mbar_wait(&drained_bar[h], tphase ^ 1);
+      const int r0 = h * 64 + wi * 16 + (lane >> 2), c0 = 2 * (lane & 3);
+#pragma unroll
+      for (int j = 0; j < BLOCK_N / 8; ++j) {
+        *reinterpret_cast<float2*>(&stg[r0 * SROW + 8 * j + c0]) = make_float2(acc[4 * j], acc[4 * j + 1]);
+        *reinterpret_cast<float2*>(&stg[(r0 + 8) * SROW + 8 * j + c0]) = make_float2(acc[4 * j + 2], acc[4 * j + 3]);
+      }
+      __syncwarp();
+      if (lane == 0) mbar_arrive(&staged_bar[h]);
+      tphase ^= 1;
+    }
+  } else {
+    regs_inc<kRegsEpilogue>();
+    sched.init(p, BLOCK_N, 0, BK);
+    const int h = role - 3;
+    const int ew = warp - 12;
+    const int wi = warp & 3;
+    const int quarter = h * 2 + (wi & 1);
+    const int half = wi >> 1;
+    const int row_in_tile = quarter * 32 + lane;
+    const int tid = threadIdx.x - 128 * role;
+    const int tiles_n = (p.N + BLOCK_N - 1) / BLOCK_N;
+    uint8_t* stg_hi = reinterpret_cast<uint8_t*>(&s_stage[ew][0][0][0]);
+    uint8_t* stg_lo = reinterpret_cast<uint8_t*>(&s_stage[ew][1][0][0]);
+    const int rsub = lane >> 1, csub = lane & 1;
+    uint32_t tphase = 0;
+    int mb, nb, kb0, kb1;
+    while (sched.next(mb, nb, kb0, kb1)) {
+      const float* srow = stg + row_in_tile * SROW + half * HALF_N;
+      const int m = mb * BLOCK_M + row_in_tile;
+      const int n0 = nb * BLOCK_N + half * HALF_N;
+      int64_t pc = 0, pe = 0;
+      int c0 = 0x7fffffff, c1 = 0x7fffffff, c2 = 0x7fffffff;
+      float v0 = 0.0f, v1 = 0.0f, v2 = 0.0f;
+      float sc = 0.0f;
+      if (m < p.M) {
+        const int64_t row = p.rows ? (int64_t)p.rows[m] : (int64_t)m;
+        const int64_t rbeg = p.indptr[row];
+        const int32_t* tp = p.tile_ptr + (int64_t)m * (kParts * tiles_n + 1) + nb * kParts + half;
+        pc = rbeg + tp[0]; pe = rbeg + tp[1];
+        if (pc < pe) { c0 = p.indices[pc]; v0 = p.values[pc]; }
+        if (pc + 1 < pe) { c1 = p.indices[pc + 1]; v1 = p.values[pc + 1]; }
+        if (pc + 2 < pe) { c2 = p.indices[pc + 2]; v2 = p.values[pc + 2]; }
+        sc = (p.weight ? p.weight[m] : 1.0f) / ((float)p.stats[DAE_STAT_SUM_W] + kEps);
+      }
+      named_bar_sync(1 + h, 128);
+      {
+        const float b = (nb * BLOCK_N + tid < p.N) ? p.bv[nb * BLOCK_N + tid] : 0.0f;
+        s_bias[h][tid] = b;
+        if (kFast) s_biasc[h][tid] = b * kLog2e;
+      }
+      mbar_wait(&staged_bar[h], tphase);
+      named_bar_sync(1 + h, 128);
+      const float inv_sc = (sc != 0.0f) ? 1.0f / sc : 0.0f;
+      const bool edge = (n0 + HALF_N > p.N);
+      float lsum = 0.0f;
+      const int m_base = mb * BLOCK_M + quarter * 32;
+      const int n_lim = edge ? p.N : 0x7fffffff;
+#pragma unroll 1
+      for (int c = 0; c < HALF_N / 16; ++c) {
+        uint32_t r[16];
+        stage_ld16(srow + c * 16, r);
+        const int nc = n0 + c * 16;
         if (m < p.M) {
-          const int64_t row = p.rows ? (int64_t)p.rows[m] : (int64_t)m;
-          const int64_t rbeg = p.indptr[row];
-          const int32_t* tp = p.tile_ptr + (int64_t)m * (kParts * tiles_n + 1) + nb * kParts + half;
-          pc = rbeg + tp[0]; pe = rbeg + tp[1];
-          if (pc < pe) { c0 = p.indices[pc]; v0 = p.values[pc]; }
-          if (pc + 1 < pe) { c1 = p.indices[pc + 1]; v1 = p.values[pc + 1]; }
-          if (pc + 2 < pe) { c2 = p.indices[pc + 2]; v2 = p.values[pc + 2]; }
-          sc = (p.weight ? p.weight[m] : 1.0f) / ((float)p.stats[DAE_STAT_SUM_W] + kEps);
+          const float* bias = &s_bias[h][half * HALF_N + c * 16];
+          uint32_t hpk[8], lpk[8];
+          bool fast_ok = false;
+          if (kFast && !edge) {
+            const float l0 = lsum;
+            fast_ok = decode_chunk_sigmoid_ce(r, &s_biasc[h][half * HALF_N + c * 16], sc, hpk, lpk, lsum);
+            if (!fast_ok) { lsum = l0; decode_chunk_generic<ACT, LOSS>(r, bias, sc, edge, n_lim, nc, hpk, lpk, lsum); }
+          } else {
+            decode_chunk_generic<ACT, LOSS>(r, bias, sc, edge, n_lim, nc, hpk, lpk, lsum);
+          }
+          uint4* sh = reinterpret_cast<uint4*>(stg_hi + lane * 48);
+          uint4* sl = reinterpret_cast<uint4*>(stg_lo + lane * 48);
+          sh[0] = make_uint4(hpk[0], hpk[1], hpk[2], hpk[3]); sh[1] = make_uint4(hpk[4], hpk[5], hpk[6], hpk[7]);
+          sl[0] = make_uint4(lpk[0], lpk[1], lpk[2], lpk[3]); sl[1] = make_uint4(lpk[4], lpk[5], lpk[6], lpk[7]);
+          while (c0 < nc + 16) {
+            const float x = v0;
+            const int j = c0 - nc;
+            __nv_bfloat16* ph = reinterpret_cast<__nv_bfloat16*>(stg_hi + lane * 48) + j;
+            __nv_bfloat16* pl = reinterpret_cast<__nv_bfloat16*>(stg_lo + lane * 48) + j;
+            float d;
+            if (kFast && fast_ok && sc != 0.0f) d = (__bfloat162float(*ph) + __bfloat162float(*pl)) * inv_sc;
+            else d = act_fast<ACT>(select16(r, j) + bias[j]);
+            const float gp = act_grad_from_y<ACT>(d);
+            float dz;
+            if (LOSS == DAE_LOSS_CE) {
+              const float a = d + kEps, b = (1.0f - d) + kEps;
+              const float la = f_lg2(a), lb = f_lg2(b);
+              lsum += lb - (x * la + (1.0f - x) * lb);
+              dz = sc * gp * ((1.0f - x) * f_rcp(b) - x * f_rcp(a));
+            } else {
+              const float e2 = x - d;
+              lsum += e2 * e2 - d * d;
+              dz = -2.0f * sc * e2 * gp;
+            }
+            const __nv_bfloat16 hb = __float2bfloat16_rn(dz);
+            *ph = hb;
+            *pl = __float2bfloat16_rn(dz - __bfloat162float(hb));
+            ++pc;
+            c0 = c1; v0 = v1; c1 = c2; v1 = v2;
+            c2 = 0x7fffffff;
+            if (pc + 2 < pe) { c2 = p.indices[pc + 2]; v2 = p.values[pc + 2]; }
+          }
         }
-        const float inv_sc = (sc != 0.0f) ? 1.0f / sc : 0.0f;
-        const bool edge = (n0 + HALF_N > p.N);
-        float lsum = 0.0f;
-        const int ew = warp - 4;
-        uint8_t* stg_hi = reinterpret_cast<uint8_t*>(&s_stage[ew][0][0][0]);
-        uint8_t* stg_lo = reinterpret_cast<uint8_t*>(&s_stage[ew][1][0][0]);
-        const int rsub = lane >> 1, csub = lane & 1;
-        const int m_base = mb * BLOCK_M + quarter * 32;
-        const int n_lim = edge ? p.N : 0x7fffffff;
-#pragma unroll 1
-        for (int c = 0; c < HALF_N / 16; ++c) {
-          uint32_t r[16];
-          stage_ld16(srow + c * 16, r);
-          const int nc = n0 + c * 16;
-          if (m < p.M) {
-            const float* bias = &s_bias[wg][half * HALF_N + c * 16];
-            uint32_t hpk[8], lpk[8];
-            bool fast_ok = false;
-            if (kFast && !edge) {
-              const float l0 = lsum;
-              fast_ok = decode_chunk_sigmoid_ce(r, &s_biasc[wg][half * HALF_N + c * 16], sc, hpk, lpk, lsum);
-              if (!fast_ok) { lsum = l0; decode_chunk_generic<ACT, LOSS>(r, bias, sc, edge, n_lim, nc, hpk, lpk, lsum); }
-            } else {
-              decode_chunk_generic<ACT, LOSS>(r, bias, sc, edge, n_lim, nc, hpk, lpk, lsum);
-            }
-            uint4* sh = reinterpret_cast<uint4*>(stg_hi + lane * 48);
-            uint4* sl = reinterpret_cast<uint4*>(stg_lo + lane * 48);
-            sh[0] = make_uint4(hpk[0], hpk[1], hpk[2], hpk[3]); sh[1] = make_uint4(hpk[4], hpk[5], hpk[6], hpk[7]);
-            sl[0] = make_uint4(lpk[0], lpk[1], lpk[2], lpk[3]); sl[1] = make_uint4(lpk[4], lpk[5], lpk[6], lpk[7]);
-            while (c0 < nc + 16) {
-              const float x = v0;
-              const int j = c0 - nc;
-              __nv_bfloat16* ph = reinterpret_cast<__nv_bfloat16*>(stg_hi + lane * 48) + j;
-              __nv_bfloat16* pl = reinterpret_cast<__nv_bfloat16*>(stg_lo + lane * 48) + j;
-              float d;
-              if (kFast && fast_ok && sc != 0.0f) d = (__bfloat162float(*ph) + __bfloat162float(*pl)) * inv_sc;
-              else d = act_fast<ACT>(select16(r, j) + bias[j]);
-              const float gp = act_grad_from_y<ACT>(d);
-              float dz;
-              if (LOSS == DAE_LOSS_CE) {
-                const float a = d + kEps, b = (1.0f - d) + kEps;
-                const float la = f_lg2(a), lb = f_lg2(b);
-                lsum += lb - (x * la + (1.0f - x) * lb);
-                dz = sc * gp * ((1.0f - x) * f_rcp(b) - x * f_rcp(a));
-              } else {
-                const float e2 = x - d;
-                lsum += e2 * e2 - d * d;
-                dz = -2.0f * sc * e2 * gp;
-              }
-              const __nv_bfloat16 hb = __float2bfloat16_rn(dz);
-              *ph = hb;
-              *pl = __float2bfloat16_rn(dz - __bfloat162float(hb));
-              ++pc;
-              c0 = c1; v0 = v1; c1 = c2; v1 = v2;
-              c2 = 0x7fffffff;
-              if (pc + 2 < pe) { c2 = p.indices[pc + 2]; v2 = p.values[pc + 2]; }
+        __syncwarp();
+        if (nc < p.ld_dz) {
+#pragma unroll
+          for (int i = 0; i < 2; ++i) {
+            const int rr = rsub + 16 * i;
+            if (m_base + rr < p.M) {
+              const int64_t off = (int64_t)(m_base + rr) * p.ld_dz + nc + csub * 8;
+              *reinterpret_cast<uint4*>(p.dz_hi + off) = *reinterpret_cast<const uint4*>(stg_hi + rr * 48 + csub * 16);
+              *reinterpret_cast<uint4*>(p.dz_lo + off) = *reinterpret_cast<const uint4*>(stg_lo + rr * 48 + csub * 16);
             }
           }
-          __syncwarp();
-          if (nc < p.ld_dz) {
-#pragma unroll
-            for (int i = 0; i < 2; ++i) {
-              const int rr = rsub + 16 * i;
-              if (m_base + rr < p.M) {
-                const int64_t off = (int64_t)(m_base + rr) * p.ld_dz + nc + csub * 8;
-                *reinterpret_cast<uint4*>(p.dz_hi + off) = *reinterpret_cast<const uint4*>(stg_hi + rr * 48 + csub * 16);
-                *reinterpret_cast<uint4*>(p.dz_lo + off) = *reinterpret_cast<const uint4*>(stg_lo + rr * 48 + csub * 16);
-              }
-            }
-          }
-          __syncwarp();
         }
-        if (m < p.M) atomicAdd(p.row_loss_part + m, (LOSS == DAE_LOSS_CE) ? lsum * 0.6931471805599453f : lsum);
+        __syncwarp();
       }
+      if (lane == 0) mbar_arrive(&drained_bar[h]);
+      tphase ^= 1;
+      if (m < p.M) atomicAdd(p.row_loss_part + m, (LOSS == DAE_LOSS_CE) ? lsum * 0.6931471805599453f : lsum);
     }
   }
-
-  if (PAIR) cluster_sync_all();
 }
 
 __global__ void decode_tile_ptr_kernel(const int64_t* __restrict__ indptr, const int32_t* __restrict__ indices,
@@ -660,15 +760,17 @@
   return fn;
 }
 
-static int make_map(CUtensorMap* m, const void* base, uint64_t inner, uint64_t outer, uint64_t ld, uint32_t box_outer) {
+static int make_map(CUtensorMap* m, const void* base, uint64_t inner, uint64_t outer, uint64_t ld, uint32_t box_outer,
+                    uint32_t box_inner = 64) {
   PFN_encodeTiled enc = get_encode();
   if (!enc) { set_error("cuTensorMapEncodeTiled entry point not found"); return DAE_ERR_CUDA; }
   cuuint64_t dims[2] = {inner, outer};
   cuuint64_t strides[1] = {ld * 2};
-  cuuint32_t box[2] = {64, box_outer};
+  cuuint32_t box[2] = {box_inner, box_outer};
   cuuint32_t estr[2] = {1, 1};
   CUresult r = enc(m, CU_TENSOR_MAP_DATA_TYPE_BFLOAT16, 2, const_cast<void*>(base), dims, strides, box, estr,
-                   CU_TENSOR_MAP_INTERLEAVE_NONE, CU_TENSOR_MAP_SWIZZLE_128B, CU_TENSOR_MAP_L2_PROMOTION_L2_256B,
+                   CU_TENSOR_MAP_INTERLEAVE_NONE, box_inner == 64 ? CU_TENSOR_MAP_SWIZZLE_128B : CU_TENSOR_MAP_SWIZZLE_64B,
+                   CU_TENSOR_MAP_L2_PROMOTION_L2_256B,
                    CU_TENSOR_MAP_FLOAT_OOB_FILL_NONE);
   if (r != CUDA_SUCCESS) { set_error("cuTensorMapEncodeTiled failed (%d): inner=%llu outer=%llu ld=%llu", (int)r,
                                      (unsigned long long)inner, (unsigned long long)outer, (unsigned long long)ld); return DAE_ERR_CUDA; }
@@ -692,7 +794,7 @@
 static int g_pair_mode = -1;
 static int g_lean = 0;
 
-template <int BLOCK_N, int STAGES, int EPI, int ACT, int LOSS, int PAIR, int MAJ>
+template <int BLOCK_N, int STAGES, int PAIR, int MAJ>
 static int launch_gemm_maj(const Operand& A, const Operand& B, GemmParams p, cudaStream_t st) {
   CUtensorMap ta_hi, ta_lo, tb_hi, tb_lo;
   int rc;
@@ -725,7 +827,7 @@
   if (PAIR) tiles_m = (tiles_m + 1) / 2;
   const int tiles_n = (p.N + BLOCK_N - 1) / BLOCK_N;
   const int kblocks = (p.K + BLOCK_K - 1) / BLOCK_K;
-  auto kern = gemm_bf16x3_kernel<BLOCK_N, STAGES, EPI, ACT, LOSS, PAIR, MAJ>;
+  auto kern = gemm_bf16x3_kernel<BLOCK_N, STAGES, PAIR, MAJ>;
   static bool attr_done[64] = {false};
   if ((rc = ensure_smem_attr(kern, smem, attr_done))) return rc;
   const int slots = PAIR ? sm_count() / 2 : sm_count();
@@ -753,15 +855,30 @@
   return DAE_OK;
 }
 
-template <int BLOCK_N, int STAGES, int EPI, int ACT, int LOSS, int PAIR>
+template <int BLOCK_N, int STAGES, int PAIR>
 static int launch_gemm(const Operand& A, const Operand& B, GemmParams p, cudaStream_t st) {
-  if (EPI == EPI_DECODE || (!A.mn_major && !B.mn_major)) return launch_gemm_maj<BLOCK_N, STAGES, EPI, ACT, LOSS, PAIR, 0>(A, B, p, st);
-  if constexpr (EPI == EPI_STORE) {
-    if (A.mn_major && !B.mn_major) return launch_gemm_maj<BLOCK_N, STAGES, EPI, ACT, LOSS, PAIR, 1>(A, B, p, st);
-    if (!A.mn_major) return launch_gemm_maj<BLOCK_N, STAGES, EPI, ACT, LOSS, PAIR, 2>(A, B, p, st);
-    return launch_gemm_maj<BLOCK_N, STAGES, EPI, ACT, LOSS, PAIR, 3>(A, B, p, st);
-  }
-  return DAE_ERR_UNSUPPORTED;
+  if (!A.mn_major && !B.mn_major) return launch_gemm_maj<BLOCK_N, STAGES, PAIR, 0>(A, B, p, st);
+  if (A.mn_major && !B.mn_major) return launch_gemm_maj<BLOCK_N, STAGES, PAIR, 1>(A, B, p, st);
+  if (!A.mn_major) return launch_gemm_maj<BLOCK_N, STAGES, PAIR, 2>(A, B, p, st);
+  return launch_gemm_maj<BLOCK_N, STAGES, PAIR, 3>(A, B, p, st);
+}
+
+template <int ACT, int LOSS>
+static int launch_decode(const Operand& A, const Operand& B, const GemmParams& p, cudaStream_t st) {
+  CUtensorMap ta_hi, ta_lo, tb_hi, tb_lo;
+  int rc;
+  if ((rc = make_map(&ta_hi, A.hi, p.K, p.M, A.ld, BLOCK_M, kDecodeBK))) return rc;
+  if ((rc = make_map(&ta_lo, A.lo, p.K, p.M, A.ld, BLOCK_M, kDecodeBK))) return rc;
+  if ((rc = make_map(&tb_hi, B.hi, p.K, p.N, B.ld, kDecodeN, kDecodeBK))) return rc;
+  if ((rc = make_map(&tb_lo, B.lo, p.K, p.N, B.ld, kDecodeN, kDecodeBK))) return rc;
+  constexpr int smem = kDecodeStages * (2 * BLOCK_M * kDecodeBK * 2 + 2 * kDecodeN * kDecodeBK * 2) + BLOCK_M * (kDecodeN + 4) * 4 + 1024;
+  auto kern = decode_fused_kernel<ACT, LOSS>;
+  static bool attr_done[64] = {false};
+  if ((rc = ensure_smem_attr(kern, smem, attr_done))) return rc;
+  const int tiles = ((p.M + BLOCK_M - 1) / BLOCK_M) * ((p.N + kDecodeN - 1) / kDecodeN);
+  const int n = tiles < sm_count() ? tiles : sm_count();
+  kern<<<n, kDecodeThreads, smem, st>>>(ta_hi, ta_lo, tb_hi, tb_lo, p);
+  return DAE_OK;
 }
 
 static bool use_pair() { return g_pair_mode == 1 && !g_lean; }
@@ -833,10 +950,10 @@
   int rc;
   const int tiles128 = tm * tn128 * k_splits, tiles64 = tm * tn64 * k_splits;
   const float cost128 = 2.0f * (float)((tiles128 + sms - 1) / sms), cost64 = 1.1f * (float)((tiles64 + sms - 1) / sms);
-  if (g_lean) rc = launch_gemm<64, 2, EPI_STORE, 0, 0, 0>(A, B, p, st);
-  else if (use_pair()) rc = launch_gemm<128, 2, EPI_STORE, 0, 0, 1>(A, B, p, st);
-  else if (!stream_k && cost64 < cost128) rc = launch_gemm<64, 3, EPI_STORE, 0, 0, 0>(A, B, p, st);
-  else rc = launch_gemm<128, 2, EPI_STORE, 0, 0, 0>(A, B, p, st);
+  if (g_lean) rc = launch_gemm<64, 2, 0>(A, B, p, st);
+  else if (use_pair()) rc = launch_gemm<128, 2, 1>(A, B, p, st);
+  else if (!stream_k && cost64 < cost128) rc = launch_gemm<64, 3, 0>(A, B, p, st);
+  else rc = launch_gemm<128, 2, 0>(A, B, p, st);
   if (rc) return rc;
   DAE_CHECK_LAUNCH("dae_gemm_bf16x3");
   return DAE_OK;
@@ -853,7 +970,7 @@
   p.C = C; p.ldc = ldc; p.n_store = N; p.special_col = -1; p.special_out = nullptr; p.a_sym_kb = kb_half;
   if (!accumulate) DAE_CUDA(cudaMemset2DAsync(C, ldc * sizeof(float), 0, (size_t)N * sizeof(float), M, (cudaStream_t)stream));
   Operand A{g_hi, g_lo, ldg, 0}, B{b_hi, b_lo, ldb, 1};
-  int rc = launch_gemm_maj<128, 2, EPI_STORE, 0, 0, 0, 6>(A, B, p, (cudaStream_t)stream);
+  int rc = launch_gemm_maj<128, 2, 0, 6>(A, B, p, (cudaStream_t)stream);
   if (rc) return rc;
   DAE_CHECK_LAUNCH("dae_gemm_sym_bf16x3");
   return DAE_OK;
@@ -892,9 +1009,7 @@
   }
   Operand A{e_hi, e_lo, lde, 0}, B{w_hi, w_lo, ldw, 0};
   int rc = 0;
-  const bool pair = (g_pair_mode == 1);
-#define DAE_DEC(ACT, LOSS) rc = pair ? launch_gemm<kDecodeN, 2, EPI_DECODE, ACT, LOSS, 1>(A, B, p, st) \
-                              : launch_gemm<kDecodeN, 2, EPI_DECODE, ACT, LOSS, 0>(A, B, p, st)
+#define DAE_DEC(ACT, LOSS) rc = launch_decode<ACT, LOSS>(A, B, p, st)
   if (loss_func == DAE_LOSS_CE) {
     if (dec_act == DAE_ACT_SIGMOID) DAE_DEC(DAE_ACT_SIGMOID, DAE_LOSS_CE);
     else if (dec_act == DAE_ACT_TANH) DAE_DEC(DAE_ACT_TANH, DAE_LOSS_CE);
```

Measured after the change: 2.139 million (median of 6 runs). +3.8%, better.
